# tenstack/batch-scheduler

Hardware: AMD Instinct MI355X
Metric: pod x node fit evals/sec (higher is better)
Workload: dtype int64; 1 GPU; cfg3/tail: 10000 pods / 2000 groups / 5000 nodes, 5 int64 lanes (cpu, mem, eph, pods, gpu), seed 20260921; stages=prefilter+filter+tally+ready, parallelism=single GPU

## Files before the change

### batch-scheduler_amd/capi.py

```python
from __future__ import annotations

import ctypes as C
import os

import numpy as np

from . import fitspec, soa

HERE = os.path.dirname(os.path.abspath(__file__))
LIB_PATH = os.path.join(os.environ.get("BS_LIB_DIR") or HERE, "libbsched.so")

KERNEL_COUNT = 8
KERNEL_PREPASS, KERNEL_LEADER, KERNEL_QUERY, KERNEL_TABLES, KERNEL_SCAN, KERNEL_RESOLVE, KERNEL_FILTER, KERNEL_TALLY = range(8)

ABI_SYMBOLS = [
    "bs_abi_version", "bs_strerror", "bs_last_error", "bs_create", "bs_destroy",
    "bs_nodes_load", "bs_fit_load", "bs_fit_build", "bs_fit_read", "bs_groups_load", "bs_groups_read", "bs_groups_apply", "bs_pods_map", "bs_pods_load",
    "bs_pods_apply", "bs_pods_count", "bs_pods_read", "bs_pods_apply_stats", "bs_filter_deny_stats", "bs_speculation_stats",
    "bs_nodes_apply", "bs_nodes_count", "bs_nodes_assume",
    "bs_cluster_fits", "bs_node_left", "bs_scan_prefix", "bs_cluster_total", "bs_filter_one", "bs_find_max_pg",
    "bs_batch_run", "bs_batch_sync", "bs_batch_read", "bs_batch_map", "bs_filter_rows_count", "bs_queue_order_load", "bs_queue_sort",
    "bs_shard_set", "bs_reduce_external", "bs_group_admit_devptr", "bs_group_admit_bind", "bs_stream", "bs_comm_unique_id", "bs_comm_init", "bs_batch_finish",
    "bs_timing_reset", "bs_timing_get", "bs_kernel_name", "bs_batch_stats_get",
    "bs_seq_run", "bs_nodes_read", "bs_first_reach_hint",
    "bs_nodes_load_flat", "bs_groups_load_flat", "bs_groups_read_flat", "bs_pods_load_flat", "bs_pods_apply_flat", "bs_pods_read_flat",
    "bs_batch_read_flat", "bs_seq_run_flat", "bs_fit_build_flat",
    "bs_bound_load", "bs_bound_count", "bs_preempt_run", "bs_bound_load_flat", "bs_preempt_run_flat",
    "bs_preempt_commit", "bs_bound_read", "bs_preempt_commit_flat",
    "bs_bound_pdb_set", "bs_preempt_pdb_read",
    "bs_bound_apply", "bs_bound_apply_flat", "bs_bound_ids", "bs_bound_dump",
    "bs_bound_nodes_apply",
    "bs_bound_apply_ex", "bs_bound_apply_ex_flat",
    "bs_pdb_load", "bs_pdb_members_append", "bs_pdb_allowed_apply", "bs_pdb_read",
    "bs_preempt_commit_gang", "bs_preempt_commit_gang_flat", "bs_preempt_gang_read",
    "bs_seq_expire", "bs_seq_expire_flat", "bs_seq_waiting_read",
    "bs_wait_load", "bs_wait_count", "bs_wait_ids", "bs_wait_read", "bs_wait_park", "bs_wait_release", "bs_wait_expire", "bs_wait_forget",
    "bs_wait_nodes_apply",
    "bs_groups_list_apply", "bs_groups_list_apply_flat",
    "bs_bound_bind",
    "bs_nominated_load", "bs_nominated_count", "bs_nominated_ids", "bs_nominated_read", "bs_nominated_apply", "bs_preempt_nominated_read",
    "bs_nominated_nodes_apply",
    "bs_preempt_cleared_read",
    "bs_seq_run_nominated", "bs_seq_run_nominated_flat", "bs_seq_nominated_read",
    "bs_seq_run_scored", "bs_seq_run_scored_flat", "bs_seq_score_read",
    "bs_seq_run_scored_nominated", "bs_seq_run_scored_nominated_flat",
]

SEQ_EXPIRE_DENY, SEQ_EXPIRE_ALL = 1, 2
WAIT_MAX = 1 << 24
NOM_MAX = 1 << 16
NOM_NONE = 0xFFFFFFFF
SCORE_WEIGHT_MAX = 65536

BS_BOUND_NODES = soa.BS_BOUND_NODES

PROTECTED_PHASES = (2, 5)


def group_protected(phases) -> np.ndarray:
    ph = np.asarray(phases, dtype=np.int64).reshape(-1)
    return np.isin(ph, PROTECTED_PHASES).astype(np.uint8)


def gang_order(pod_group, priority) -> np.ndarray:
    grp = np.asarray(pod_group, np.int64).reshape(-1)
    pri = np.asarray(priority, np.int64).reshape(-1)
    assert grp.shape == pri.shape
    first: dict = {}
    rank = np.zeros(grp.shape[0], np.int64)
    for i in range(grp.shape[0]):
        key = (int(pri[i]), int(grp[i])) if grp[i] >= 0 else (int(pri[i]), -1 - i)
        rank[i] = first.setdefault(key, i)
    return np.lexsort((np.arange(grp.shape[0]), rank, -pri)).astype(np.int64)


def gang_need(groups, waiting=None) -> np.ndarray:
    mm = np.asarray(groups.min_member, np.int64).reshape(-1)
    w = np.zeros_like(mm) if waiting is None else np.asarray(waiting, np.int64).reshape(-1)
    assert w.shape == mm.shape
    return np.clip(mm - np.asarray(groups.status_scheduled, np.int64).reshape(-1) - w, 0, None).astype(np.uint32)


class BsError(RuntimeError):
    def __init__(self, status: int, where: str, detail: str = ""):
        self.status = status
        super().__init__(f"{where}: status {status}" + (f" ({detail})" if detail else ""))


class Config(C.Structure):
    _fields_ = [("abi_version", C.c_uint32), ("device", C.c_int32), ("scalar_lanes", C.c_uint32),
                ("eph_gate", C.c_uint32), ("enable_timing", C.c_uint32), ("reserved", C.c_uint32 * 3)]


class NodeDelta(C.Structure):
    _fields_ = [("kind", C.c_uint32), ("index", C.c_uint32),
                ("allocatable", C.c_int64 * soa.MAX_LANES), ("requested", C.c_int64 * soa.MAX_LANES),
                ("allocatable_present", C.c_uint32), ("requested_present", C.c_uint32), ("flags", C.c_uint32),
                ("fit_default", C.c_uint32), ("n_fit_exceptions", C.c_uint32), ("fit_exceptions", C.c_uint32 * 8)]


class NodeRequest(C.Structure):
    _fields_ = [("index", C.c_uint32), ("requested_present", C.c_uint32), ("requested", C.c_int64 * soa.MAX_LANES)]


DELTA_UPDATE, DELTA_APPEND, DELTA_REMOVE = 0, 1, 2

# ... 24 lines not shown


class SeqExpireOut(C.Structure):
    _fields_ = [("n_groups", C.c_uint32), ("n_pods", C.c_uint32), ("group_cap", C.c_uint32), ("group", C.POINTER(C.c_uint32)),
                ("group_pods", C.POINTER(C.c_uint32)), ("group_earlier", C.POINTER(C.c_uint32)), ("pod_cap", C.c_uint32),
                ("pod", C.POINTER(C.c_uint32)), ("node", C.POINTER(C.c_uint32))]


_lib = None


class GroupsListDelta(C.Structure):
    _fields_ = [("n_remove", C.c_uint32), ("remove", C.POINTER(C.c_uint32)), ("n_update", C.c_uint32), ("update", C.POINTER(C.c_uint32)),
                ("rows", soa.GroupsStruct), ("n_append", C.c_uint32)]


class GroupsListOut(C.Structure):
    _fields_ = [("g_new", C.c_uint32), ("n_pods_missing", C.c_uint32), ("n_bound_missing", C.c_uint32), ("n_wait_dropped", C.c_uint32),
                ("wait_cap", C.c_uint32), ("wait_id", C.POINTER(C.c_uint32)), ("wait_node", C.POINTER(C.c_uint32)), ("wait_group", C.POINTER(C.c_int32))]


def load_library(path: str | None = None):
    global _lib
    if _lib is not None and path is None:
        return _lib
    p = path or LIB_PATH
    if not os.path.exists(p):
        raise BsError(-2, "load_library", f"{p} not built: run `python __graft_entry__.py build` (hipcc, gfx950)")
    L = C.CDLL(p)
    vp, u32, i32, u8 = C.c_void_p, C.c_uint32, C.c_int32, C.c_uint8
    P = C.POINTER
    L.bs_abi_version.restype = u32
    L.bs_strerror.restype = C.c_char_p
    L.bs_strerror.argtypes = [C.c_int]
    L.bs_last_error.restype = C.c_char_p
    L.bs_last_error.argtypes = [vp]
    L.bs_kernel_name.restype = C.c_char_p
    L.bs_kernel_name.argtypes = [u32]
    L.bs_create.argtypes = [P(Config), P(vp)]
    L.bs_destroy.argtypes = [vp]
    L.bs_nodes_load.argtypes = [vp, P(soa.NodesStruct)]
    L.bs_fit_load.argtypes = [vp, u32, P(u32)]
    L.bs_fit_build.argtypes = [vp, P(fitspec.NodeLabelsStruct), P(fitspec.FitTemplatesStruct)]
    L.bs_fit_read.argtypes = [vp, P(u32)]
    L.bs_groups_load.argtypes = [vp, P(soa.GroupsStruct)]
    L.bs_groups_read.argtypes = [vp, P(soa.GroupsStruct)]
    L.bs_groups_apply.argtypes = [vp, P(soa.GroupDelta), u32]
    L.bs_filter_rows_count.argtypes = [vp, P(u32)]
    L.bs_pods_load.argtypes = [vp, P(soa.PodsStruct)]
    L.bs_pods_map.argtypes = [vp, u32, P(soa.PodsStruct)]
    L.bs_pods_apply.argtypes = [vp, P(soa.PodsDeltaStruct)]
    L.bs_pods_count.argtypes = [vp, P(u32)]
    L.bs_pods_apply_stats.argtypes = [vp, P(C.c_uint64), P(C.c_uint64)]
    L.bs_filter_deny_stats.argtypes = [vp, P(C.c_uint64)]
    L.bs_speculation_stats.argtypes = [vp, P(C.c_uint64), P(C.c_uint64)]
    L.bs_pods_read.argtypes = [vp, P(soa.PodsOutStruct)]
    L.bs_queue_order_load.argtypes = [vp, u32, P(u32)]
    L.bs_queue_sort.argtypes = [vp, u32, P(i32), P(i32), P(C.c_int64), P(u32)]
    L.bs_nodes_apply.argtypes = [vp, P(NodeDelta), u32]
    L.bs_nodes_count.argtypes = [vp, P(u32)]
    L.bs_nodes_assume.argtypes = [vp, P(NodeRequest), u32]
    L.bs_cluster_fits.argtypes = [vp, u32, C.c_float, P(C.c_int64), u32, P(u8), P(u32)]
    L.bs_node_left.argtypes = [vp, u32, C.c_float, P(C.c_int64), P(u32)]
    L.bs_scan_prefix.argtypes = [vp, u32, C.c_float, P(C.c_int64), P(u32), P(u32), P(u32)]
    L.bs_cluster_total.argtypes = [vp, u32, P(C.c_int64), P(u32)]
    L.bs_filter_one.argtypes = [vp, i32, P(C.c_int64), u32, i32, u32, P(u8), P(u8)]
    L.bs_find_max_pg.argtypes = [vp, P(i32), P(u32), P(u8)]
    L.bs_batch_run.argtypes = [vp, u32]
    L.bs_batch_sync.argtypes = [vp]
    L.bs_batch_read.argtypes = [vp, P(soa.BatchOutStruct)]
    L.bs_batch_map.argtypes = [vp, P(soa.BatchViewStruct)]
    L.bs_shard_set.argtypes = [vp, u32, u32]
    L.bs_group_admit_devptr.argtypes = [vp, P(vp), P(u32)]
    L.bs_reduce_external.argtypes = [vp, u32]
    L.bs_first_reach_hint.argtypes = [vp, u32]
    L.bs_group_admit_bind.argtypes = [vp, vp]
    L.bs_stream.argtypes = [vp, P(vp)]
    L.bs_comm_unique_id.argtypes = [P(u8)]
    L.bs_comm_init.argtypes = [vp, P(u8), u32, u32]
    L.bs_batch_finish.argtypes = [vp]
    L.bs_timing_reset.argtypes = [vp]
    L.bs_timing_get.argtypes = [vp, P(Timing)]
    L.bs_batch_stats_get.argtypes = [vp, P(BatchStats)]
    L.bs_seq_run.argtypes = [vp, u32, P(SeqOut)]
    L.bs_nodes_read.argtypes = [vp, P(C.c_int64), P(u32)]
    L.bs_bound_load.argtypes = [vp, P(soa.BoundStruct)]
    L.bs_bound_count.argtypes = [vp, P(u32)]
    L.bs_preempt_run.argtypes = [vp, u32, u32, P(u32), P(i32), P(u8), u32, P(soa.PreemptOutStruct)]
    L.bs_bound_load_flat.argtypes = [vp, u32, P(u32), P(i32), P(C.c_int64), P(i32), P(C.c_int64), P(u32)]
    L.bs_preempt_run_flat.argtypes = [vp, u32, u32, P(u32), P(i32), P(u8), u32, P(i32), P(u32), P(u32), P(u32), P(i32), P(C.c_int64), P(C.c_int64)]
    L.bs_preempt_commit.argtypes = [vp, u32, u32, P(u32), P(i32), P(u8), u32, u32, P(soa.PreemptOutStruct)]
    L.bs_bound_read.argtypes = [vp, P(u32), P(u32)]
    L.bs_bound_pdb_set.argtypes = [vp, u32, P(u8)]
    L.bs_bound_apply.argtypes = [vp, P(soa.BoundDeltaStruct), P(u32)]
    L.bs_bound_apply_flat.argtypes = [vp, u32, P(u32), u32, P(u32), P(i32), P(C.c_int64), P(i32), P(C.c_int64), P(u32), P(u8), P(u32)]
    L.bs_bound_apply_ex.argtypes = [vp, P(soa.BoundDeltaStruct), u32, P(u32)]
    L.bs_bound_apply_ex_flat.argtypes = [vp, u32, u32, P(u32), u32, P(u32), P(i32), P(C.c_int64), P(i32), P(C.c_int64), P(u32), P(u8), P(u32)]
    L.bs_bound_ids.argtypes = [vp, P(u32)]
    L.bs_bound_nodes_apply.argtypes = [vp, u32, P(u32), P(u32), u32, P(u32), P(u32)]
    L.bs_bound_dump.argtypes = [vp, P(i32), P(C.c_int64), P(i32), P(C.c_int64), P(u32), P(u8)]
    L.bs_preempt_pdb_read.argtypes = [vp, u32, P(u32)]
    L.bs_pdb_load.argtypes = [vp, u32, P(i32), u32, P(u32), P(u32)]
    L.bs_pdb_members_append.argtypes = [vp, u32, u32, P(u32), P(u32)]
    L.bs_pdb_allowed_apply.argtypes = [vp, u32, P(u32), P(i32)]
    L.bs_pdb_read.argtypes = [vp, P(u32), P(u32), P(i32), P(u32)]
    L.bs_preempt_commit_flat.argtypes = [vp, u32, u32, P(u32), P(i32), P(u8), u32, u32, P(i32), P(u32), P(u32), P(u32), P(i32), P(C.c_int64),
                                         P(C.c_int64)]
    L.bs_preempt_commit_gang.argtypes = [vp, u32, u32, P(u32), P(i32), P(u8), P(u32), u32, u32, P(soa.PreemptOutStruct)]
    L.bs_preempt_commit_gang_flat.argtypes = [vp, u32, u32, P(u32), P(i32), P(u8), P(u32), u32, u32, P(i32), P(u32), P(u32), P(u32), P(i32),
                                              P(C.c_int64), P(C.c_int64)]
    L.bs_preempt_gang_read.argtypes = [vp, u32, P(u8), u32, P(u32)]
    L.bs_seq_expire.argtypes = [vp, u32, P(u32), u32, P(SeqExpireOut)]
    L.bs_seq_expire_flat.argtypes = [vp, u32, P(u32), u32, u32, P(u32), P(u32), P(u32), u32, P(u32), P(u32), P(u32)]
    L.bs_seq_waiting_read.argtypes = [vp, u32, P(i32)]
    L.bs_wait_load.argtypes = [vp, u32, P(u32), P(i32), P(C.c_int64), P(u32)]
    L.bs_wait_count.argtypes = [vp, P(u32)]
    L.bs_wait_ids.argtypes = [vp, P(u32)]
    L.bs_wait_read.argtypes = [vp, P(u32), P(u32), P(i32), P(C.c_int64), P(u32)]
    L.bs_wait_park.argtypes = [vp, u32, P(u32), P(u32), P(u32), P(u32)]
    L.bs_wait_release.argtypes = [vp, u32, P(u32), u32, P(u32), P(u32), P(u32), P(u32)]
    L.bs_wait_expire.argtypes = [vp, u32, P(u32), u32, u32, P(u32), P(u32), P(u32), P(u32), P(u32)]
    L.bs_wait_forget.argtypes = [vp, u32, P(u32), P(u32)]
    L.bs_wait_nodes_apply.argtypes = [vp, u32, P(u32), P(u32), u32, P(u32), P(u32), P(i32), P(u32)]
    L.bs_groups_list_apply.argtypes = [vp, P(GroupsListDelta), P(GroupsListOut)]
    L.bs_groups_list_apply_flat.argtypes = [vp, u32, P(u32), u32, P(u32), u32, P(u32), P(u32), P(u32), P(u8), P(u32), P(C.c_int64), P(u32), P(C.c_uint64),
                                            u32, u32, P(u32), P(u32), P(i32), P(u32)]
    L.bs_nominated_load.argtypes = [vp, u32, P(u32), P(i32), P(C.c_int64), P(u32)]
    L.bs_nominated_count.argtypes = [vp, P(u32)]
    L.bs_nominated_ids.argtypes = [vp, P(u32)]
    L.bs_nominated_read.argtypes = [vp, P(u32), P(u32), P(i32), P(C.c_int64), P(u32)]
    L.bs_nominated_apply.argtypes = [vp, u32, P(u32), u32, P(u32), P(u32), P(i32), P(u32)]
    L.bs_preempt_nominated_read.argtypes = [vp, u32, P(u32)]
    L.bs_preempt_cleared_read.argtypes = [vp, u32, P(u32), P(u32), P(i32), P(u32), P(u32)]
    L.bs_nominated_nodes_apply.argtypes = [vp, u32, P(u32), P(u32), u32, P(u32), P(u32), P(i32), P(u32)]
    L.bs_bound_bind.argtypes = [vp, u32, P(u32), u32, P(u32), P(i32), P(C.c_int64), P(u8), P(u32), P(u32)]
    L.bs_seq_run_nominated.argtypes = [vp, u32, u32, P(i32), P(u32), P(SeqOut)]
    L.bs_seq_run_nominated_flat.argtypes = [vp, u32, u32, P(i32), P(u32), P(u8), P(u32), P(i32), P(i32), u32, P(u32), P(u32), P(C.c_int64), P(C.c_int64),
                                            P(C.c_int64), P(u8)]
    L.bs_seq_nominated_read.argtypes = [vp, u32, P(u32), P(u32), P(u32), P(u32)]
    L.bs_seq_run_scored.argtypes = [vp, u32, P(SeqScore), P(SeqOut)]
    L.bs_seq_run_scored_flat.argtypes = [vp, u32, u32, u32, u32, P(u8), P(u32), P(i32), P(i32), u32, P(u32), P(u32), P(C.c_int64), P(C.c_int64),
                                         P(C.c_int64), P(u8)]
    L.bs_seq_score_read.argtypes = [vp, u32, P(u32), P(u32)]
    L.bs_seq_run_scored_nominated.argtypes = [vp, u32, u32, P(i32), P(u32), P(SeqScore), P(SeqOut)]
    L.bs_seq_run_scored_nominated_flat.argtypes = [vp, u32, u32, P(i32), P(u32), u32, u32, u32, P(u8), P(u32), P(i32), P(i32), u32, P(u32), P(u32), P(C.c_int64),
                                                   P(C.c_int64), P(C.c_int64), P(u8)]
    for name in ABI_SYMBOLS:
        fn = getattr(L, name)
        if fn.restype is C.c_int:
            fn.restype = C.c_int
    if path is None:
        _lib = L
    return L


def _i64p(a):
    return a.ctypes.data_as(C.POINTER(C.c_int64))


def _u32p(a):
    return a.ctypes.data_as(C.POINTER(C.c_uint32))


class Context:

    def __init__(self, scalar_lanes: int = 0, eph_gate: int = 1, device: int = 0, enable_timing: int = 0):
# ... 725 lines not shown
    def bound_nodes_apply(self, kind, index, dropped_cap: int = 0):
        kv = np.ascontiguousarray(np.asarray(kind, np.uint32).reshape(-1))
        iv = np.ascontiguousarray(np.asarray(index, np.uint32).reshape(-1))
        assert kv.size == iv.size
        ids = np.zeros(max(int(dropped_cap), 1), np.uint32)
        nd = C.c_uint32()
        self._chk(self._lib.bs_bound_nodes_apply(self._h, int(kv.size), _u32p(kv) if kv.size else None, _u32p(iv) if iv.size else None,
                                                 int(dropped_cap), _u32p(ids) if dropped_cap else None, C.byref(nd)), "bs_bound_nodes_apply")
        return int(nd.value), ids[: min(int(nd.value), int(dropped_cap))].copy()

    def pdb_load(self, allowed, member_off, member, b: int | None = None):
        al = np.ascontiguousarray(allowed, np.int32).reshape(-1)
        off = np.ascontiguousarray(member_off, np.uint32).reshape(-1)
        mem = np.ascontiguousarray(member, np.uint32).reshape(-1)
        b = max(off.size - 1, 0) if b is None else int(b)
        self._chk(self._lib.bs_pdb_load(self._h, int(al.size), al.ctypes.data_as(C.POINTER(C.c_int32)) if al.size else None, b,
                                        _u32p(off) if off.size else None, _u32p(mem) if mem.size else None), "bs_pdb_load")

    def pdb_members_append(self, first_id: int, member_off, member):
        off = np.ascontiguousarray(member_off, np.uint32).reshape(-1)
        mem = np.ascontiguousarray(member, np.uint32).reshape(-1)
        self._chk(self._lib.bs_pdb_members_append(self._h, int(first_id), max(off.size - 1, 0), _u32p(off) if off.size else None,
                                                  _u32p(mem) if mem.size else None), "bs_pdb_members_append")

    def pdb_allowed_apply(self, index, value):
        ix = np.ascontiguousarray(index, np.uint32).reshape(-1)
        va = np.ascontiguousarray(value, np.int32).reshape(-1)
        assert ix.size == va.size
        self._chk(self._lib.bs_pdb_allowed_apply(self._h, int(ix.size), _u32p(ix) if ix.size else None,
                                                 va.ctypes.data_as(C.POINTER(C.c_int32)) if va.size else None), "bs_pdb_allowed_apply")

    def pdb_read(self) -> dict:
        n, cov = C.c_uint32(0), C.c_uint32(0)
        self._chk(self._lib.bs_pdb_read(self._h, C.byref(n), C.byref(cov), None, None), "bs_pdb_read")
        nodes = C.c_uint32(0)
        self._chk(self._lib.bs_nodes_count(self._h, C.byref(nodes)), "bs_nodes_count")
        al, nv = np.zeros(max(n.value, 1), np.int32), np.zeros(max(nodes.value, 1), np.uint32)
        self._chk(self._lib.bs_pdb_read(self._h, None, None, al.ctypes.data_as(C.POINTER(C.c_int32)), _u32p(nv)), "bs_pdb_read")
        return dict(n_pdb=int(n.value), covered=int(cov.value), allowed=al[: n.value], node_violating=nv[: nodes.value])

    def bound_dump(self) -> dict:
        b = self.bound_count()
        n = max(b, 1)
        prio, start, grp = np.zeros(n, np.int32), np.zeros(n, np.int64), np.zeros(n, np.int32)
        req, pres, pdb = np.zeros((self.L, n), np.int64), np.zeros(n, np.uint32), np.zeros(n, np.uint8)
        self._chk(self._lib.bs_bound_dump(self._h, prio.ctypes.data_as(C.POINTER(C.c_int32)), _i64p(start), grp.ctypes.data_as(C.POINTER(C.c_int32)),
                                          _i64p(req), _u32p(pres), pdb.ctypes.data_as(C.POINTER(C.c_uint8))), "bs_bound_dump")
        return dict(priority=prio[:b], start_ns=start[:b], group=grp[:b], req=req[:, :b], req_present=pres[:b], pdb=pdb[:b])

    def set_shard(self, rank: int, nranks: int):
        self._chk(self._lib.bs_shard_set(self._h, rank, nranks), "bs_shard_set")

    def reduce_external(self, on: bool = True):
        self._chk(self._lib.bs_reduce_external(self._h, 1 if on else 0), "bs_reduce_external")

    def first_reach_hint(self, local_index: int):
        self._chk(self._lib.bs_first_reach_hint(self._h, int(local_index) & 0xFFFFFFFF), "bs_first_reach_hint")

    def admit_devptr(self):
        p, n = C.c_void_p(), C.c_uint32(0)
        self._chk(self._lib.bs_group_admit_devptr(self._h, C.byref(p), C.byref(n)), "bs_group_admit_devptr")
        return int(p.value or 0), int(n.value)

    def bind_admit(self, dptr: int | None):
        self._chk(self._lib.bs_group_admit_bind(self._h, C.c_void_p(dptr or 0)), "bs_group_admit_bind")

    def stream(self) -> int:
        p = C.c_void_p()
        self._chk(self._lib.bs_stream(self._h, C.byref(p)), "bs_stream")
        return int(p.value or 0)

    def comm_init(self, uid: bytes, rank: int, nranks: int):
        buf = (C.c_uint8 * 128).from_buffer_copy(uid)
        self._chk(self._lib.bs_comm_init(self._h, buf, rank, nranks), "bs_comm_init")

    def timing_reset(self):
        self._chk(self._lib.bs_timing_reset(self._h), "bs_timing_reset")

    def timing(self) -> dict:
        t = Timing()
        self._chk(self._lib.bs_timing_get(self._h, C.byref(t)), "bs_timing_get")
        return {self._lib.bs_kernel_name(i).decode(): (float(t.total_ms[i]), int(t.launches[i])) for i in range(KERNEL_COUNT)}

    def stats_arm(self):
        s = BatchStats()
        self._chk(self._lib.bs_batch_stats_get(self._h, C.byref(s)), "bs_batch_stats_get")

    def stats(self, stages: int = soa.STAGE_ALL) -> dict:
        self.stats_arm()
        self.run(stages)
        self.sync()
        return self.stats_read()

    def stats_read(self) -> dict:
        s = BatchStats()
        self._chk(self._lib.bs_batch_stats_get(self._h, C.byref(s)), "bs_batch_stats_get")
        return {k: int(getattr(s, k)) for k, _ in BatchStats._fields_}


def comm_unique_id() -> bytes:
    lib = load_library()
    buf = (C.c_uint8 * 128)()
    rc = lib.bs_comm_unique_id(buf)
    if rc != 0:
        raise BsError(rc, "bs_comm_unique_id")
    return bytes(buf)
```

### batch-scheduler_amd/csrc/bs_ctx.hpp

```cpp
#pragma once
#include <rccl/rccl.h>

#include <algorithm>
#include <cstring>
#include <functional>
#include <string>
#include <vector>

#include "bs_carve.hpp"
#include "bs_hostmem.hpp"
#include "bs_kernels.hpp"
#include "bs_lanes.hpp"
#include "bs_layouts.hpp"
#include "bs_pod_ranges.hpp"
#include "bs_preempt_clear_list.hpp"

namespace bs {

struct EventPair { hipEvent_t a, b; uint32_t id; };

inline size_t align256(size_t x) { return (x + 255) & ~(size_t)255; }
template <class T>
T* at(T* p, size_t n) { return p ? p + n : nullptr; }

// ... 128 lines not shown
  uint64_t n_applies = 0, n_rederives = 0;
  OutLayout olay;

  DevBuf d_first_elig, d_first_owner, d_first_reject, d_first_pod, d_cap_epoch;
  DevBuf d_epoch, d_nepochs, d_leader_epoch, d_panic_epoch;
  DevBuf d_tcode, d_stage, d_leader_raw, d_first_row, d_first_row64, d_scan_rec, d_feas_rec, d_chunk_rec, d_qreq_s, d_qflags_s, d_qpos;
  DevBuf d_needed, d_qcount, d_ticket, d_desc;
  bool scratch_armed = false;
  bool side_ready = false;
  DevBuf d_tables, d_kp, d_stats, d_fparams, d_fflags, d_chunk_tot, d_blk_scratch, d_gmax, d_chunk_kp;
  DevBuf d_cls_slots, d_cls_rep, d_cls_id, d_qtab_s, d_fu_slot, d_uparams, d_uflags, d_uclaim, d_fu_bitmap, d_fu_feas;
  DevBuf d_nodew;
  bool batch_void = false;
  uint32_t tp_tmin = 768;
  bool no_nodew = false;
  uint32_t slot_keep = 0xFFFFFFFFu;
  uint32_t cls_cap = 0, hash_keep = 0x7FFFFFFFu, n_nominres = 0, scan_slots_cap = 0, filter_slots_cap = 0;
  DevBuf d_fl_bitmap, d_admit, d_ready, d_gcount, d_admit64, d_own_start;
  bool owner_ready = false;
  DevBuf d_order_rank, d_sort;
  uint32_t order_g = 0;
  DevBuf d_gstat, d_pair_next, d_pair_firstq, d_first_reach, d_qstamp_s, d_fast_reject, d_epoch_group;
  bool pairs_ready = false;
  bool bitmap_valid = false;
  bool last_fast = false;
  bool batch_since_pods = false;
  size_t off_hfeas = 0, off_htag = 0;
  uint32_t hstride = 0;
  int32_t host_tag = 0;
  bool last_host_out = false;
  uint32_t no_fast = 0;
  DevBuf d_run_of_epoch, d_run_leader, d_gslot, d_gfirstq;
  bool epochs_ready = false, einfo_pending = false;
  int32_t einfo_tag = 0;
  uint32_t h_R = 0, h_eflags = 0, no_epoch = 0;
  uint32_t last_chain = 0;
  uint32_t last_rows = 0;
  DevBuf d_sq;
  DevBuf d_seq;
  bool seq_wait_valid = false;
  Piece<unsigned long long> seq_o_wait;
  Piece<uint32_t> seq_o_head, seq_o_nwait;
  Piece<int32_t> seq_o_node;
  bool seq_nom_valid = false;
  std::vector<uint32_t> seq_nom_id, seq_nom_pod, seq_nom_node;
  DevBuf d_seq_score;
  bool seq_score_valid = false;
  uint32_t seq_score_p = 0;
  DevBuf d_sexp;
  DevBuf d_sexp_nodes;
  uint32_t sexp_n = 0, sexp_l = 0;
  bool sexp_clean = false;
  bool have_wait = false;
  uint32_t wait_w = 0, wait_ids = 0;
  uint32_t wait_n = 0, wait_g = 0;
  DevBuf d_wait[2];
  uint32_t wait_cap[2] = {0, 0};
  uint32_t wait_cur = 0;
  DevBuf d_wait_scr;
  DevBuf d_wait_nodes;
  DevBuf d_wait_gmark, d_wait_imark;
  bool wait_nodes_clean = false, wait_gmark_clean = false, wait_imark_clean = false;
  uint32_t table_slots = 0, table_mcap = 0;

  uint32_t rank = 0, nranks = 1;
  bool reduce_external = false;
  uint32_t* ext_admit = nullptr;
  int32_t sop_leader0 = -1;
  uint32_t last_stages = 0;
  uint64_t batch_seq = 0;
  uint32_t stamp_ctr = 1, key_seq = 1;
  bool rekey_pending = false;
  bool batch_pending_finish = false;
  bool groups_launch_pending = false;
  DeltaPack pending_dp{};
  uint32_t no_fuse_final = 0;
  uint32_t tp_filter = 6;
  uint32_t tp_share = 0;
  uint32_t tp_fwaves = 0;
  bool filter_waves_env = false;
  uint32_t tp_split = 0;
  int fused_blocks_resident = -1;
  int step_a_resident[2] = {-1, -1};
  uint32_t step_a_form = 3;
  bool step_a_on = true;
  uint32_t step_shares = 8;
  uint32_t test_timeout_after = 0;
  uint32_t test_pc_chunk_nodes = 0;
  uint32_t tk_pods = 0, tk_tab = 0;
  uint32_t tk_p1 = 0, tk_done = 0;
  bool pod_ranges_on = true;
  bool ranges_valid = false;
  uint32_t nranges = 0;
  PodRanges h_ranges;
  std::vector<uint32_t> h_pod_ranges;
  DevBuf d_pod_ranges;
  bool last_step_a = false;
  uint32_t scan_share_override = 0, no_fuse_filter = 0, early_forced = 0, target_waves = 8192, filter_waves = 8192, collect_stats = 0;
  uint32_t general_waves = 4096;
  bs_batch_stats stats{};

  std::vector<EventPair> events;
  size_t events_used = 0;
  bs_timing timing{};

  void* rccl_handle = nullptr;
  void* comm = nullptr;
  decltype(&ncclAllReduce) rccl_allreduce = nullptr;
  decltype(&ncclCommDestroy) rccl_destroy = nullptr;
  uint32_t launches = 0;
  DevBuf d_fd_event, d_fd_in, d_fd_flag;
  bool fd_on = false;
  bool fd_active = false;
  uint32_t first_reach_hint = 0xFFFFFFFFu;
  bool fd_unsynced = false;
  bool fd_in_live = false;
  uint32_t fd_iter = 0, fd_stages = 0, fd_seq_inv = 0;
  uint64_t n_fd_reruns = 0;
  bool have_bound = false;
  uint32_t bound_b = 0, bound_n = 0;
  int32_t bound_max_group = -1;
  DevBuf d_bound, d_pre;
  DevBuf d_bound2;
  BoundLayout blay{};
  uint32_t bound_ids = 0;
  std::vector<uint32_t> pre_npv;
  bool have_pre_npv = false;
  std::vector<uint8_t> gang_voided;
  std::vector<uint32_t> gang_placed;
  bool have_gang = false;
  bool have_pdb = false;
  uint32_t pdb_n = 0, pdb_covered = 0, pdb_members = 0;
  DevBuf d_pdb_allowed, d_pdb_moff, d_pdb_member;
  bool have_nom = false;
  uint32_t nom_w = 0, nom_ids = 0;
  uint32_t nom_n = 0;
  DevBuf d_nom[2];
  uint32_t nom_cap[2] = {0, 0};
  uint32_t nom_ncap[2] = {0, 0};
  uint32_t nom_cur = 0;
  std::vector<uint32_t> nom_live;
  std::vector<uint32_t> pre_nom;
  bool have_pre_nom = false;
  ClearedRows pre_clr;

  Stream stream;
  Stream stream3;
  Event ev_query, ev_filter;
  PinnedBuf<int32_t> h_info{PinWait::None, hipHostMallocMapped | hipHostMallocCoherent};
  PinnedBuf<> h_gstage{PinWait::Event};
  PinnedBuf<> h_glstage{PinWait::Stream};
  PinnedBuf<> h_stage{PinWait::Event};
  PinnedBuf<> h_dstage{PinWait::Stream};
  PinnedBuf<> h_nstage{PinWait::Event};
  PinnedBuf<> h_pdbstage{PinWait::Stream};
  PinnedBuf<> h_rstage;
  PinnedBuf<> h_hout{PinWait::None, hipHostMallocMapped | hipHostMallocCoherent};
  PinnedBuf<uint64_t> h_hrows{PinWait::None, hipHostMallocMapped | hipHostMallocCoherent};
};

inline int32_t hinfo_get(const bs_ctx* c, HInfo w) { return static_cast<volatile const int32_t*>(c->h_info.p)[w]; }
inline void hinfo_set(bs_ctx* c, HInfo w, int32_t v) { static_cast<volatile int32_t*>(c->h_info.p)[w] = v; }
inline int32_t* hinfo_at(const bs_ctx* c, HInfo w) { return c->h_info.p ? c->h_info.p + w : nullptr; }

#define HIPCHK(ctx, call)                                                                         \
  do {                                                                                            \
    hipError_t _e = (call);                                                                       \
    if (_e != hipSuccess) {                                                                       \
      (ctx)->last_error = std::string(#call) + ": " + hipGetErrorString(_e);                      \
      return BS_ERR_HIP;                                                                          \
    }                                                                                             \
  } while (0)
#define LAUNCHCHK(ctx, id)                                                                         \
  do {                                                                                             \
    hipError_t _e = hipGetLastError();                                                             \
    if (_e != hipSuccess) {                                                                        \
      (ctx)->last_error = std::string("launch of kernel group '") + kKernelNames[id] + "': " + hipGetErrorString(_e); \
      return BS_ERR_HIP;                                                                           \
    }                                                                                              \
  } while (0)
// ... 1 lines not shown
```

### batch-scheduler_amd/csrc/bs_fast.hpp

```cpp
#pragma once

#include "bs_kernels.hpp"
#include "bs_filter_t.hpp"

#ifdef BS_NT_TABLES
#define BS_TBL_STORE(p, v) __builtin_nontemporal_store((v), (p))
#else
#define BS_TBL_STORE(p, v) (*(p) = (v))
#endif
namespace bs {

template <bool INL = false>
__device__ __forceinline__ void arm_tally(const GroupsDev& gr, const BatchDev& b, const BatchParams& prm, uint32_t i, uint32_t nthreads);

__device__ __forceinline__ const uint8_t* range_glocal(const BatchDev& b) { return reinterpret_cast<const uint8_t*>(b.pod_ranges); }
__device__ __forceinline__ const uint32_t* range_start(const BatchDev& b, uint32_t G) { return b.pod_ranges + (G + 3u) / 4u; }
__device__ __forceinline__ const uint32_t* range_lfirst(const BatchDev& b, uint32_t G, uint32_t pod_blocks) { return range_start(b, G) + pod_blocks + 1u; }
__device__ __forceinline__ bool range_local_on(const BatchDev& b, const BatchParams& prm) {
  return b.pod_ranges && prm.do_tally && prm.do_ready && !prm.filter_deny;
}

#if BS_EMIT_MAIN
__global__ void k_pods_prep(unsigned long long* tables, uint32_t ntab, uint32_t* gstat, uint32_t ngstat, uint32_t* kcount, uint32_t* gcount, uint32_t G) {
  const uint32_t t = blockIdx.x * blockDim.x + threadIdx.x, nt = gridDim.x * blockDim.x;
// ... 466 lines not shown
    LeaderPre lp{};
    const bool have = gr.g != 0 && leaders[s] >= 0;
    if (have) leader_pre_load(gr, leaders[s], sh, lp);
    Res ms;
    res_zero(ms, sh);
    if (have && lp.have_mr) res_add(ms, lp.mr, sh, gate);
    uint32_t ff = (have && lp.have_mr) ? 1u : 0u;
#pragma unroll
    for (uint32_t q = 0; q < BS_MAX_SCALARS; ++q)
      if (q < sh.S() && (ms.present & (1u << q)) && ms.v[4 + q] != 0) ff |= 2u;
    const unsigned long long holds = __ballot(l[0] >= ms.v[0] && l[1] >= ms.v[1] && l[2] >= ms.v[2] && l[3] >= ms.v[3]);
    if (stores) {
      b.nodew[nodew_pair(stride, s, w)] = ok;
      b.nodew[nodew_pair(stride, s, w) + 1] = ~holds;
    }
    if (blk == 0 && threadIdx.x == 0) {
#pragma unroll
      for (int j = 0; j < 4; ++j) b.nodew[nodew_ref_lane(stride, s, j)] = (uint64_t)ms.v[j];
      b.nodew[nodew_ref_flags(stride, s)] = ff;
    }
  }
}

template <int TS>
__global__ __launch_bounds__(kTblChunk) void k_fast_query_tables(PodsDev pods, GroupsDev gr, NodesDev nd, BatchDev b, BatchDev bt, BatchParams prm,
                                                                 const TableDesc* forced, uint32_t nchunks, uint32_t query_blocks) {
  BS_STAMP(1, 0);
  if (blockIdx.x < query_blocks) fast_query_thread<TS>(pods, gr, b, prm, blockIdx.x * kTblChunk + threadIdx.x, query_blocks * kTblChunk);
  else if (blockIdx.x < query_blocks + nchunks) tables_local_fast<TS>(nd, bt, prm, forced, blockIdx.x - query_blocks);
  else node_words_block<TS>(gr, nd, b, prm, blockIdx.x - query_blocks - nchunks);
  BS_STAMP(1, 7);
}

template <int NL>
__device__ __forceinline__ unsigned long long rows_cover(unsigned long long m, const int64_t (&a)[BS_MAX_LANES], const int64_t (&r)[BS_MAX_LANES]) {
  asm volatile("s_mov_b64 exec, %[m]\n\tv_cmpx_ge_i64 vcc, %[a0], %[r0]\n\tv_cmpx_ge_i64 vcc, %[a1], %[r1]\n\tv_cmpx_ge_i64 vcc, %[a2], %[r2]\n\t"
               "v_cmpx_ge_i64 vcc, %[a3], %[r3]\n\ts_mov_b64 %[m], exec\n\ts_mov_b64 exec, -1"
               : [m] "+s"(m)
               : [a0] "v"(a[0]), [r0] "v"(r[0]), [a1] "v"(a[1]), [r1] "v"(r[1]), [a2] "v"(a[2]), [r2] "v"(r[2]), [a3] "v"(a[3]), [r3] "v"(r[3])
               : "vcc");
#pragma unroll
  for (int j = 4; j < NL; ++j)
    asm volatile("s_mov_b64 exec, %[m]\n\tv_cmpx_ge_i64 vcc, %[a], %[r]\n\ts_mov_b64 %[m], exec\n\ts_mov_b64 exec, -1" : [m] "+s"(m) : [a] "v"(a[j]), [r] "v"(r[j]) : "vcc");
  return m;
}
#ifndef BS_SCAN_BALLOT
#define BS_SCAN_BALLOT 1
#endif
constexpr uint32_t kSpinBound = 1u << 18;
__device__ __forceinline__ void test_chaos_delay() {
#ifdef BS_TEST_CHAOS
  uint32_t h = (blockIdx.x + 1u) * 2654435761u ^ (uint32_t)wall_clock64() * 40503u;
  h ^= h >> 15; h *= 2246822519u; h ^= h >> 13;
  for (uint32_t s = 0; s < (h & 15u); ++s) __builtin_amdgcn_s_sleep(127);
#endif
}
__device__ __forceinline__ bool step_wait(const uint32_t* word, uint32_t base, uint32_t need, int32_t* h_err) {
  uint32_t spins = 0;
  while ((uint32_t)(ld_agent(word) - base) < need) {
    __builtin_amdgcn_s_sleep(1);
    if (++spins > kSpinBound) { if (h_err) __hip_atomic_store(h_err, 1, __ATOMIC_RELAXED, __HIP_MEMORY_SCOPE_SYSTEM); return false; }
  }
  return true;
}
constexpr uint32_t kScanRecChunks = 64;
constexpr uint32_t kFeasRecGroups = 32;
constexpr uint32_t kRecStride = 32;
constexpr uint32_t kTkSlots = 32, kTkTab = 48, kTkP1 = 64, kTkDone = 64 + 16 * 16, kTkWays = 16, kTkWords = 64 + 2 * 16 * 16;
__device__ __forceinline__ void spread_add(uint32_t* words, uint32_t who) {
  (void)__hip_atomic_fetch_add(&words[16u * (who % kTkWays)], 1u, __ATOMIC_RELAXED, __HIP_MEMORY_SCOPE_AGENT);
}
__device__ __forceinline__ bool spread_wait(const uint32_t* words, uint32_t base, uint32_t need, int32_t* h_err) {
  uint32_t spins = 0;
  for (;;) {
    uint32_t v = lane_id() < (int)kTkWays ? ld_agent(&words[16u * (uint32_t)lane_id()]) : 0u;
#pragma unroll
    for (int o = 1; o < (int)kTkWays; o <<= 1) v += (uint32_t)__shfl_xor((int)v, o);
    v = (uint32_t)__builtin_amdgcn_readfirstlane((int)v);
    if ((uint32_t)(v - base) >= need) return true;
    __builtin_amdgcn_s_sleep(4);
    if (++spins > kSpinBound) { if (h_err && lane_id() == 0) __hip_atomic_store(h_err, 1, __ATOMIC_RELAXED, __HIP_MEMORY_SCOPE_SYSTEM); return false; }
  }
}
template <int TS, bool REGS = false>
__device__ __forceinline__ void table_scan_block(const NodesDev& nd, const BatchDev& b, const BatchParams& prm, const TableDesc* forced, uint32_t chunk, uint32_t nchunks,
                                                 uint32_t share, uint32_t nshares, uint32_t pod_blocks, uint32_t tk_pods0, uint32_t tk_tab0, const GroupsDev& gr,
                                                 const int64_t* ckeys, const uint32_t* cpres, uint32_t kcap, bool direct = false, uint32_t forced_cls = 0) {
  __shared__ unsigned long long s_wtot[BS_MAX_LANES][4];
  __shared__ uint32_t s_kp[BS_MAX_SCALARS];
  __shared__ unsigned long long s_off[BS_MAX_LANES];
  __shared__ uint32_t s_kpg[BS_MAX_SCALARS];
  __shared__ int64_t s_req[kStepSlotsMax][BS_MAX_LANES];
  __shared__ uint32_t s_qf[kStepSlotsMax];
  __shared__ uint32_t s_first[kStepSlotsMax];
  BS_STAMP(2, 0);
  const Shape<TS> sh(prm.S);
  const uint32_t L = sh.L(), S = sh.S(), LP = prm.LP;
  const uint32_t k = chunk * kTblChunk + threadIdx.x;
  const bool in_range = REGS ? k < nd.n : k < nd.m;
  const uint32_t n = REGS ? (in_range ? k : 0u) : (in_range ? nd.kmap[k] : 0u);
  const TableDesc d = REGS ? TableDesc{forced_cls, 0.7f} : *forced;
  const uint32_t fw = nd.fit[(size_t)d.cls * nd.fit_words + (n >> 5)];
  const uint8_t fl = nd.flags[n];
  const bool valid = in_range && (!REGS || !(fl & BS_NODE_SKIP_MASK));
  const uint32_t ap = nd.apres[n], rp = nd.rpres[n];
  int64_t al[BS_MAX_LANES], rq[BS_MAX_LANES];
#pragma unroll
  for (uint32_t j = 0; j < BS_MAX_LANES; ++j) {
    if (j < L) {
      al[j] = nd.alloc[(size_t)j * nd.stride + n];
      rq[j] = nd.req[(size_t)j * nd.stride + n];
    }
  }
  const uint32_t K = prm.k_host ? prm.k_host : *b.kclass;
  const uint32_t per = (K + nshares - 1u) / nshares, s_lo = share * per, s_hi = min(K, s_lo + per);
  Res raw;
  int32_t leader0 = -1;
  uint8_t panic0 = 0;
  LeaderPre lp0{};
  if constexpr (REGS) {
    const uint32_t cc = s_lo + threadIdx.x < s_hi ? s_lo + threadIdx.x : 0u;
#pragma unroll
    for (uint32_t j = 0; j < BS_MAX_LANES; ++j)
      if (j < L) raw.v[j] = ckeys[(size_t)j * kcap + cc];
    raw.present = cpres[cc];
    leader0 = b.leader_epoch[0];
    panic0 = b.panic_epoch[0];
    if (gr.g) leader_pre_load(gr, leader0, sh, lp0);
  }
  const bool fit = valid && ((fw >> (n & 31u)) & 1u) && !(fl & BS_NODE_TAINT_ERR);
  const uint32_t pres = fit ? (ap & rp) : 0u;
  if (threadIdx.x < BS_MAX_SCALARS) s_kp[threadIdx.x] = BS_INF;
  for (uint32_t t = threadIdx.x; t < kStepSlotsMax; t += kTblChunk) s_first[t] = BS_INF;
  unsigned long long incl[BS_MAX_LANES];
  const int w = wave_id();
#pragma unroll
  for (uint32_t j = 0; j < BS_MAX_LANES; ++j) {
    incl[j] = 0;
    if (j < L) {
      const bool live = fit && (j < 4 || (pres & (1u << (j - 4)))) && !(j == BS_LANE_EPH && !prm.eph_gate);
      const unsigned long long left = live ? (unsigned long long)wsub(scale_f32(al[j], d.pct), rq[j]) : 0ull;
      incl[j] = wave_incl_scan_add_u64(left);
      if (lane_id() == 63) s_wtot[j][w] = incl[j];
    }
  }
  __syncthreads();
#pragma unroll
  for (uint32_t s2 = 0; s2 < BS_MAX_SCALARS; ++s2) {
    if (s2 < S) {
      const unsigned long long mk = __ballot(valid && (pres & (1u << s2)));
      if (mk && lane_id() == 0) atomicMin(&s_kp[s2], chunk * kTblChunk + (uint32_t)(threadIdx.x & ~63u) + (uint32_t)(__ffsll((long long)mk) - 1));
    }
  }
#pragma unroll
  for (uint32_t j = 0; j < BS_MAX_LANES; ++j) {
    if (j < L) {
      unsigned long long off = 0, tot = 0;
#pragma unroll
      for (int i = 0; i < 4; ++i) {
        const unsigned long long x = s_wtot[j][i];
        if (i < w) off += x;
        tot += x;
      }
      incl[j] += off;
      if (threadIdx.x == 0 && share == 0) {
        if constexpr (REGS) {
          const unsigned long long tag = (unsigned long long)prm.seq_inv << 32;
          st_pub<true>(&b.chunk_rec[(size_t)chunk * kRecStride + 2u * j], tag | (uint32_t)tot);
          st_pub<true>(&b.chunk_rec[(size_t)chunk * kRecStride + 2u * j + 1u], tag | (uint32_t)(tot >> 32));
        } else {
          st_pub<true>(&b.chunk_tot[(size_t)chunk * 16 + j], tot);
        }
      }
    }
  }
  __syncthreads();
  __shared__ uint32_t s_ok;
  if constexpr (REGS) {
    if (share == 0 && threadIdx.x < S) st_pub<true>(&b.chunk_rec[(size_t)chunk * kRecStride + 16u + threadIdx.x], ((unsigned long long)prm.seq_inv << 32) | s_kp[threadIdx.x]);
    BS_STAMP(2, 1);
  } else {
    if (share == 0 && threadIdx.x < 16) st_pub<true>(&b.chunk_kp[(size_t)chunk * 16 + threadIdx.x], threadIdx.x < BS_MAX_SCALARS ? s_kp[threadIdx.x] : BS_INF);
    asm volatile("s_waitcnt vmcnt(0)" ::: "memory");
    __syncthreads();
    BS_STAMP(2, 1);
    if (threadIdx.x == 0 && share == 0) (void)__hip_atomic_fetch_add(&b.ticket[kTkTab], 1u, __ATOMIC_RELAXED, __HIP_MEMORY_SCOPE_AGENT);
  }
  if constexpr (REGS) {
    const uint32_t t = s_lo + threadIdx.x;
    if (t < s_hi) {
      uint32_t qf = 0x80000000u;
      Res q;
      res_zero(q, sh);
      if (leader0 >= 0 && !panic0) {
        Res cur;
        res_zero(cur, sh);
        res_add(cur, raw, sh, prm.eph_gate);
        qf = class_scan_query(cur, lp0, sh, prm.eph_gate, q);
      }
      s_qf[threadIdx.x] = qf;
#pragma unroll
      for (uint32_t j = 0; j < BS_MAX_LANES; ++j)
        if (j < L) s_req[threadIdx.x][j] = q.v[j];
    }
  }
  if constexpr (!REGS) {
    if (threadIdx.x == 0) s_ok = (step_wait(&b.ticket[kTkTab], tk_tab0, nchunks, b.h_err) && step_wait(&b.ticket[kTkSlots], tk_pods0, pod_blocks, b.h_err)) ? 1u : 0u;
    __syncthreads();
    BS_STAMP(2, 2);
    if (!s_ok) return;
  }
  {
    const uint32_t ch = (uint32_t)lane_id();
    unsigned long long cv[BS_MAX_LANES];
    uint32_t ckp[BS_MAX_SCALARS];
    if constexpr (REGS) {
      if (w == 0) {
        const uint32_t tagw = prm.seq_inv;
        const unsigned long long* rec = b.chunk_rec + (size_t)(ch < nchunks ? ch : 0u) * kRecStride;
        bool ok = false;
        for (uint32_t spins = 0;; ++spins) {
          unsigned long long lo[BS_MAX_LANES], hi[BS_MAX_LANES], kw[BS_MAX_SCALARS];
#pragma unroll
          for (uint32_t j = 0; j < BS_MAX_LANES; ++j)
            if (j < L) { lo[j] = ld_agent64(&rec[2u * j]); hi[j] = ld_agent64(&rec[2u * j + 1u]); }
// ... 47 lines not shown
    if (w == 0) {
#pragma unroll
      for (uint32_t j = 0; j < BS_MAX_LANES; ++j) {
        if (j < L) {
          const unsigned long long incl_c = wave_incl_scan_add_u64(cv[j]);
          const unsigned long long mine = bcast64(incl_c - cv[j], (int)(chunk & 63u));
          if (ch == 0) s_off[j] = mine;
        }
      }
#pragma unroll
      for (uint32_t s2 = 0; s2 < BS_MAX_SCALARS; ++s2) {
        if (s2 < S) {
          const uint32_t mn = wave_min_u32(ckp[s2]);
          if (ch == 0) s_kpg[s2] = mn;
        }
      }
    }
    if (!REGS && t < s_hi) {
      if (stp != prm.stamp || tab != 0) qf = 0x80000000u;
      s_qf[threadIdx.x] = qf;
#pragma unroll
      for (uint32_t j = 0; j < BS_MAX_LANES; ++j)
        if (j < L) s_req[threadIdx.x][j] = (int64_t)rv[j];
    }
  }
  __syncthreads();
  if constexpr (REGS) {
    if (!s_ok) return;
  }
  int64_t fin[BS_MAX_LANES];
  uint32_t keyrow = 0;
#pragma unroll
  for (uint32_t j = 0; j < BS_MAX_LANES; ++j) {
    fin[j] = 0;
    if (j < L) fin[j] = (int64_t)(incl[j] + s_off[j]);
  }
#pragma unroll
  for (uint32_t s2 = 0; s2 < BS_MAX_SCALARS; ++s2)
    if (s2 < S && k >= s_kpg[s2]) keyrow |= 1u << s2;
  BS_STAMP(2, 3);
  const uint32_t nmine = s_hi > s_lo ? s_hi - s_lo : 0u;
  const uint32_t smask = S ? ((1u << S) - 1u) : 0u;
  const uint32_t row0 = chunk * kTblChunk + ((uint32_t)w << 6);
  for (uint32_t t0 = 0; t0 < nmine; t0 += 4u) {
    uint32_t qf[4];
    int64_t r[4][BS_MAX_LANES];
#pragma unroll
    for (uint32_t u = 0; u < 4; ++u) {
      const uint32_t t = min(t0 + u, nmine - 1u);
      qf[u] = t0 + u < nmine ? s_qf[t] : 0x80000000u;
#pragma unroll
      for (uint32_t j = 0; j < BS_MAX_LANES; ++j) r[u][j] = j < L ? s_req[t][j] : 0;
    }
#pragma unroll
    for (uint32_t u = 0; u < 4; ++u) {
      const uint32_t nab = ~(qf[u] >> 16) & smask;
      unsigned long long m = (qf[u] & 0x80000000u) ? 0ull : __ballot(valid && (nab & ~keyrow) == 0u);
      static_assert(TS >= 0 && TS <= 4, "k_fast_step_a is instantiated for 0..4 scalar lanes (bs_step_geom.hpp: step_a_possible)");
#if BS_SCAN_BALLOT
#pragma unroll
      for (uint32_t j = 0; j < 4u + (uint32_t)TS; ++j) m &= __ballot(fin[j] >= r[u][j]);
#else
      m = rows_cover<4 + TS>(m, fin, r[u]);
#endif
      if (m && lane_id() == 0) atomicMin(&s_first[t0 + u], row0 + (uint32_t)(__ffsll((long long)m) - 1));
    }
  }
  __syncthreads();
  BS_STAMP(2, 4);
  if constexpr (REGS) {
    if (direct) {
      for (uint32_t t = threadIdx.x; t < nmine; t += kTblChunk)
        st_pub<true>(&b.scan_rec[(size_t)chunk * kStepSlotsMax + s_lo + t], ((unsigned long long)prm.seq_inv << 32) | s_first[t]);
    } else {
      for (uint32_t t = threadIdx.x; t < nmine; t += kTblChunk)
        if (s_first[t] != BS_INF) atomicMin(&b.first_row64[s_lo + t], ((unsigned long long)prm.seq_inv << 32) | s_first[t]);
    }
    BS_STAMP(2, 7);
    return;
  }
  for (uint32_t t = threadIdx.x; t < nmine; t += kTblChunk) {
    if (s_first[t] == BS_INF) continue;
    atomicMin(&b.first_row[s_lo + t], s_first[t]);
  }
  BS_STAMP(2, 7);
}

__device__ __forceinline__ void step_filter_split(uint32_t K, uint32_t W, uint32_t target_waves, uint32_t& tiles, uint32_t& bpw, uint32_t& nchunk) {
  tiles = (2u * K + 63u) / 64u;
  uint32_t nsplit = max(1u, target_waves / max(tiles, 1u));
  nsplit = min(nsplit, max((W + 1u) / 2u, 1u));
  bpw = max(2u, (((W + nsplit - 1u) / nsplit + 1u) / 2u) * 2u);
  nchunk = (W + bpw - 1u) / bpw;
  if ((nchunk + 3u) / 4u > kFeasRecGroups) {
    bpw = ((W + 4u * kFeasRecGroups - 1u) / (4u * kFeasRecGroups) + 1u) / 2u * 2u;
    nchunk = (W + bpw - 1u) / bpw;
  }
}
template <int TS>
__device__ __forceinline__ void step_filter_block(const GroupsDev& gr, const NodesDev& nd, const BatchDev& b, const BatchParams& prm, const int64_t* ckeys,
                                                  const uint32_t* cpres, uint32_t kcap, uint32_t target_waves, uint32_t ustride, uint32_t bx, uint32_t nblocks,
                                                  bool direct, uint32_t tk_slots0, uint32_t slot_producers) {
  __shared__ uint32_t s_cnt[4][64];
  BS_STAMP_AT(4, 0, bx);
  const Shape<TS> sh(prm.S);
  const uint32_t gate = prm.eph_gate, K = prm.k_host ? prm.k_host : (uint32_t)__builtin_amdgcn_readfirstlane((int)*b.kclass), U = 2u * K;
  const uint32_t W = (nd.n + 63u) / 64u;
  if (!U || !W) return;
  uint32_t tiles, bpw, nchunk;
  step_filter_split(K, W, target_waves, tiles, bpw, nchunk);
  const uint32_t groups = (nchunk + 3u) / 4u;
  const int32_t leader0 = b.leader_epoch[0];
  LeaderPre lp0{}, lp1{};
  const bool two = prm.sop_leader0 >= 0 && prm.sop_leader0 != leader0;
  if (gr.g) {
    leader_pre_load(gr, leader0, sh, lp0);
    if (two) leader_pre_load(gr, prm.sop_leader0, sh, lp1); else lp1 = lp0;
  }
  bool waited = false;
  for (uint32_t bi = bx; bi < tiles * groups; bi += nblocks) {
    const uint32_t tile = bi % tiles, group = bi / tiles, chunk = group * 4u + (uint32_t)wave_id();
    const uint32_t src = tile * 64u + (uint32_t)lane_id();
    const bool second = src >= K;
    const uint32_t c = src < U ? (second ? src - K : src) : 0u;
    uint32_t cnt = 0;
    if (chunk < nchunk) {
      Res raw;
#pragma unroll
      for (uint32_t j = 0; j < BS_MAX_LANES; ++j)
        if (j < sh.L()) raw.v[j] = ckeys[(size_t)j * kcap + c];
      raw.present = cpres[c];
      Res cur;
      res_zero(cur, sh);
      res_add(cur, raw, sh, gate);
      LeaderPre lp = lp0;
      if (second) lp = lp1;
      const bool on = src < U && (second ? prm.sop_leader0 >= 0 : leader0 >= 0) && lp.have_mr;
      int64_t R[4], M[4];
      const uint32_t ff = filter_slot_values(cur, lp, sh, gate, R, M);
      filter_item<2, 4, true, true>(nd, b, U, ustride, tile, chunk * bpw, min(W, chunk * bpw + bpw), 0u,
                                    on ? (ff | ((uint32_t)BS_FL_EVALUATED << 8)) : ((uint32_t)BS_FL_NOT_RUN << 8), R, M, &cnt);
    }
    s_cnt[wave_id()][lane_id()] = cnt;
    BS_STAMP_AT(4, 1, bx);
    if (direct && b.h_rows) asm volatile("s_waitcnt vmcnt(0)" ::: "memory");
    __syncthreads();
    BS_STAMP_AT(4, 2, bx);
    if (wave_id() == 0 && src < U) {
      const uint32_t sum = s_cnt[0][lane_id()] + s_cnt[1][lane_id()] + s_cnt[2][lane_id()] + s_cnt[3][lane_id()];
      if (direct) {
        st_pub<true>(&b.feas_rec[(size_t)group * (2u * kStepSlotsMax) + src], ((unsigned long long)prm.seq_inv << 32) | sum);
      } else {
        if (!waited) { (void)step_wait(&b.ticket[kTkSlots], tk_slots0, slot_producers, b.h_err); waited = true; }
        if (sum) atomicAdd(&b.fu_feas[src], sum);
      }
    }
    __syncthreads();
  }
  BS_STAMP_AT(4, 7, bx);
}

template <int TS>
__device__ __forceinline__ void class_slots_block(const GroupsDev& gr, const BatchDev& b, const BatchParams& prm, const int64_t* ckeys, const uint32_t* cpres,
                                                  uint32_t kcap, uint32_t blk, bool zero_feas) {
  const Shape<TS> sh(prm.S);
#ifdef BS_TEST_OLD_ZERO
// ... 361 lines not shown
    else
      tally_tail<true>(gr, b, prm, grouped, grouped ? (uint32_t)gi0 : 0u, admit, nblocks);
  }
  BS_STAMP(3, 7);
}

template <int S>
__global__ __launch_bounds__(256) void k_fast_scan_filter(PodsDev pods, NodesDev nd, BatchDev bt, BatchParams prm, uint32_t m, uint32_t jcap,
                                                          uint32_t scan_blocks, uint32_t filter_waves, uint32_t ustride) {
  __shared__ int64_t s_rows[4][64][4 + S];
  if (blockIdx.x < scan_blocks)
    scan_loop<S, true, 1>(bt, prm, m, jcap, 0u, 0u, 1u, blockIdx.x, scan_blocks, s_rows[wave_id()]);
  else
    filter_loop<2>(pods, nd, bt, filter_waves, 1u, ustride, prm.collect_stats, blockIdx.x - scan_blocks, gridDim.x - scan_blocks, prm.stamp, 2u * prm.k_host);
}
template <int S>
__global__ __launch_bounds__(256) void k_fast_scan(BatchDev bt, BatchParams prm, uint32_t m, uint32_t jcap) {
  __shared__ int64_t s_rows[4][64][4 + S];
  scan_loop<S, true, 1>(bt, prm, m, jcap, 0u, 0u, 1u, blockIdx.x, gridDim.x, s_rows[wave_id()]);
}
template <int PU, bool DB>
__global__ __launch_bounds__(256) void k_fast_filter(PodsDev pods, NodesDev nd, BatchDev bt, BatchParams prm, uint32_t filter_waves, uint32_t ustride) {
  filter_loop<2, PU, DB>(pods, nd, bt, filter_waves, 1u, ustride, prm.collect_stats, blockIdx.x, gridDim.x, prm.stamp, 2u * prm.k_host);
}
#if BS_EMIT_FAST
__global__ __launch_bounds__(256) __attribute__((amdgpu_waves_per_eu(7))) void k_fast_filter_w7(PodsDev pods, NodesDev nd, BatchDev bt, BatchParams prm, uint32_t filter_waves,
                                                                                                uint32_t ustride) {
  filter_loop<2, 2, false>(pods, nd, bt, filter_waves, 1u, ustride, prm.collect_stats, blockIdx.x, gridDim.x, prm.stamp, 2u * prm.k_host);
}
#endif
#if BS_EMIT_FAST
__global__ __launch_bounds__(256) void k_fast_filter_t(NodesDev nd, BatchDev bt, BatchParams prm, uint32_t filter_waves, uint32_t ustride, uint32_t by_tile) {
  filter_loop_t<false>(nd, bt, filter_waves, ustride, prm.collect_stats, blockIdx.x, gridDim.x, prm.stamp, 2u * prm.k_host, by_tile);
}
#endif
template <int S>
__global__ __launch_bounds__(256) __attribute__((amdgpu_waves_per_eu(S <= 1 ? 4 : 1))) void k_fast_scan_filter_t(NodesDev nd, BatchDev bt, BatchParams prm, uint32_t m, uint32_t jcap, uint32_t scan_blocks,
                                                            uint32_t filter_waves, uint32_t ustride, uint32_t form) {
  __shared__ int64_t s_rows[4][64][4 + S];
  const uint32_t filter_first = form & 1u, by_tile = form & 2u;
  const uint32_t filter_blocks = gridDim.x - scan_blocks;
  const bool is_scan = filter_first ? blockIdx.x >= filter_blocks : blockIdx.x < scan_blocks;
  BS_STAMP(2, 0);
  if (is_scan)
    scan_loop<S, true, 1>(bt, prm, m, jcap, 0u, 0u, 1u, filter_first ? blockIdx.x - filter_blocks : blockIdx.x, scan_blocks, s_rows[wave_id()]);
  else
    filter_loop_t<true>(nd, bt, filter_waves, ustride, prm.collect_stats, filter_first ? blockIdx.x : blockIdx.x - scan_blocks, filter_blocks, prm.stamp, 2u * prm.k_host, by_tile);
  BS_STAMP(2, 7);
}
#if BS_EMIT_MAIN
__global__ __launch_bounds__(256) void k_fast_final(PodsDev pods, GroupsDev gr, NodesDev nd, BatchDev b, BatchParams prm, uint32_t query_blocks) {
  fast_final_block(pods, gr, nd, b, prm, query_blocks, blockIdx.x, gridDim.x, 0u);
}
#endif

template <int S>
__global__ __launch_bounds__(256) void k_fast_scan_filter_final(PodsDev pods, GroupsDev gr, NodesDev nd, BatchDev b, BatchDev bt, BatchParams prm, uint32_t m,
                                                                uint32_t jcap, uint32_t scan_blocks, uint32_t filter_blocks, uint32_t filter_waves,
                                                                uint32_t ustride, uint32_t query_blocks) {
  __shared__ int64_t s_rows[4][64][4 + S];
  const uint32_t producers = scan_blocks + filter_blocks;
  test_chaos_delay();
#ifdef BS_TEST_LATE_ROLE_B
  {
    const int role = blockIdx.x < scan_blocks ? 0 : blockIdx.x < producers ? 1 : 2;
    if (role == BS_TEST_LATE_ROLE_B) for (int spin = 0; spin < 20; ++spin) __builtin_amdgcn_s_sleep(127);
  }
#endif
  if (blockIdx.x < producers) {
    BS_STAMP(2, 0);
    if (blockIdx.x < scan_blocks)
      scan_loop<S, true, 2>(bt, prm, m, jcap, 0u, 0u, 1u, blockIdx.x, scan_blocks, s_rows[wave_id()]);
    else
      filter_loop<2>(pods, nd, bt, filter_waves, 1u, ustride, prm.collect_stats, blockIdx.x - scan_blocks, filter_blocks, prm.stamp, 2u * prm.k_host);
    asm volatile("s_waitcnt vmcnt(0)" ::: "memory");
    __syncthreads();
    if (threadIdx.x == 0) (void)__hip_atomic_fetch_add(&b.ticket[1], 1u, __ATOMIC_RELAXED, __HIP_MEMORY_SCOPE_AGENT);
    BS_STAMP(2, 7);
    return;
  }
  fast_final_block(pods, gr, nd, b, prm, query_blocks, blockIdx.x - producers, gridDim.x - producers, producers);
}

template <int TS, bool WHOLE>
__global__ __launch_bounds__(kTblChunk) void k_fast_step_a(PodsDev pods, GroupsDev gr, NodesDev nd, BatchDev b, BatchDev bt, BatchParams prm, const TableDesc* forced,
                                                           uint32_t nchunks, uint32_t query_blocks, uint32_t nshares, uint32_t filter_blocks, uint32_t filter_waves,
                                                           uint32_t ustride, uint32_t tk_pods0, uint32_t tk_tab0, uint32_t param_blocks, const int64_t* ckeys,
                                                           const uint32_t* cpres, uint32_t kcap, uint32_t tk_p1, uint32_t tk_done, uint32_t forced_cls) {
  BS_STAMP(1, 0);
  test_chaos_delay();
  const uint32_t tb = nchunks * nshares;
#ifdef BS_TEST_LATE_ROLE
  {
    const int role = blockIdx.x < query_blocks ? 0 : blockIdx.x < query_blocks + param_blocks ? 1 : blockIdx.x < query_blocks + param_blocks + tb ? 2 : 3;
    if (role == BS_TEST_LATE_ROLE) for (int spin = 0; spin < 20; ++spin) __builtin_amdgcn_s_sleep(127);
  }
#endif
  const uint32_t producers = param_blocks ? param_blocks : query_blocks;
  const bool direct = query_blocks <= kGatherDirectBlocks;
  if (blockIdx.x < query_blocks) {
    if constexpr (WHOLE) {
      const uint32_t p0 = b.pod_ranges ? range_start(b, gr.g)[blockIdx.x] : blockIdx.x * kTblChunk;
      const uint32_t p1 = b.pod_ranges ? range_start(b, gr.g)[blockIdx.x + 1u] : pods.p;
      fast_query_thread<TS, false, false, true>(pods, gr, b, prm, p0 + threadIdx.x, query_blocks * kTblChunk, p1, blockIdx.x * kTblChunk + threadIdx.x);
      asm volatile("s_waitcnt vmcnt(0)" ::: "memory");
      __syncthreads();
      if (threadIdx.x == 0) spread_add(&b.ticket[kTkP1], blockIdx.x);
      fast_final_block<true>(pods, gr, nd, b, prm, query_blocks, blockIdx.x, query_blocks, nchunks, tk_p1, filter_waves, tk_done, tb + filter_blocks, p0, p1);
    } else if (param_blocks) {
      fast_query_thread<TS, false, false>(pods, gr, b, prm, blockIdx.x * kTblChunk + threadIdx.x, query_blocks * kTblChunk);
    } else {
      fast_query_thread<TS, true>(pods, gr, b, prm, blockIdx.x * kTblChunk + threadIdx.x, query_blocks * kTblChunk);
      BS_STAMP(1, 4);
      asm volatile("s_waitcnt vmcnt(0)" ::: "memory");
      __syncthreads();
      BS_STAMP(1, 5);
      if (threadIdx.x == 0) (void)__hip_atomic_fetch_add(&b.ticket[kTkSlots], 1u, __ATOMIC_RELAXED, __HIP_MEMORY_SCOPE_AGENT);
    }
  } else if (blockIdx.x < query_blocks + param_blocks) {
    class_slots_block<TS>(gr, b, prm, ckeys, cpres, kcap, blockIdx.x - query_blocks, !(WHOLE && direct));
  } else if (blockIdx.x < query_blocks + param_blocks + tb) {
    const uint32_t x = blockIdx.x - query_blocks - param_blocks;
    table_scan_block<TS, WHOLE>(nd, bt, prm, forced, x / nshares, nchunks, x % nshares, nshares, producers, tk_pods0, tk_tab0, gr, ckeys, cpres, kcap, direct, forced_cls);
    if constexpr (WHOLE) {
      if (!direct) {
        asm volatile("s_waitcnt vmcnt(0)" ::: "memory");
        __syncthreads();
        if (threadIdx.x == 0) spread_add(&b.ticket[kTkDone], blockIdx.x);
      }
    }
  } else if constexpr (WHOLE) {
    step_filter_block<TS>(gr, nd, bt, prm, ckeys, cpres, kcap, filter_waves, ustride, blockIdx.x - query_blocks - param_blocks - tb, filter_blocks, direct, tk_pods0, producers);
    if (!direct) {
      asm volatile("s_waitcnt vmcnt(0)" ::: "memory");
      __syncthreads();
      if (threadIdx.x == 0) spread_add(&b.ticket[kTkDone], blockIdx.x);
    }
  } else {
    __shared__ uint32_t s_go;
    if (threadIdx.x == 0) {
      s_go = step_wait(&b.ticket[kTkSlots], tk_pods0, producers, b.h_err) ? 1u : 0u;
      __builtin_amdgcn_fence(__ATOMIC_ACQUIRE, "agent");
    }
    __syncthreads();
    if (!s_go) return;
    filter_loop<2>(pods, nd, bt, filter_waves, 1u, ustride, prm.collect_stats, blockIdx.x - query_blocks - param_blocks - tb, filter_blocks, prm.stamp, 2u * prm.k_host);
  }
  BS_STAMP(1, 7);
}


template <int TS>
__global__ __launch_bounds__(kTblChunk) void k_tables_local_nofix(NodesDev nd, BatchDev b, BatchParams prm, uint32_t nchunks, uint32_t cstride,
                                                                  uint32_t gstride) {
  const uint32_t slot = blockIdx.x;
  if (!b.needed[slot]) return;
  BatchDev bt = b;
  bt.tables = b.tables + (size_t)slot * prm.mcap * prm.LP;
  bt.kp = b.kp + (size_t)slot * 16;
  bt.chunk_tot = b.chunk_tot + (size_t)slot * cstride * 16;
  bt.chunk_kp = b.chunk_kp + (size_t)slot * cstride * 16;
  bt.gmax = b.gmax + (size_t)slot * gstride * prm.LP;
  const TableDesc d = table_desc(slot, prm.C, nullptr);
  tables_local_fast<TS>(nd, bt, prm, &d, blockIdx.y);
}

#if BS_EMIT_MAIN
__global__ __launch_bounds__(kLeaderBlock) void k_leader_scan(GroupsDev gr, BatchDev b) {
  __shared__ unsigned long long s_w[kLeaderBlock / 64];
  __shared__ uint32_t s_p[kLeaderBlock / 64];
  __shared__ unsigned long long s_carry;
  __shared__ uint32_t s_pcarry, s_nexact, s_exact[64];
  const uint32_t E1 = *b.nepochs;
  auto key_of = [&](uint32_t g, bool& panic) -> unsigned long long {
    if (gr.flags[g] & BS_GROUP_SCHEDULED_LATCH) return 0ull;
    const uint32_t f = leader_finished(gr, g, panic);
    return (((unsigned long long)f + 1ull) << 31) | (unsigned long long)(0x7FFFFFFFu - g);
  };
  unsigned long long k0 = 0;
  bool p0 = false;
  for (uint32_t g = threadIdx.x; g < gr.g; g += kLeaderBlock)
    if (b.cap_epoch[g] == 0u) { const unsigned long long k = key_of(g, p0); k0 = k > k0 ? k : k0; }
  {
    const unsigned long long m = block_max_u64(k0, s_w);
    const unsigned long long anyp = __ballot(p0);
    if (lane_id() == 0) s_p[wave_id()] = anyp ? 1u : 0u;
    __syncthreads();
    if (threadIdx.x == 0) {
      uint32_t pp = 0;
      for (int w = 0; w < kLeaderBlock / 64; ++w) pp |= s_p[w];
      s_carry = m;
      s_pcarry = pp;
      s_nexact = 0;
    }
    __syncthreads();
  }
  for (uint32_t base = 0; base < E1; base += kLeaderBlock) {
    const uint32_t e = base + threadIdx.x;
    unsigned long long k = 0;
    bool pn = false;
    if (e >= 1 && e < E1) k = key_of(b.epoch_group[e], pn);
    uint32_t pv = pn ? 1u : 0u;
#pragma unroll
    for (int o = 1; o < 64; o <<= 1) {
      const unsigned long long u = __shfl_up(k, o);
      const uint32_t q = (uint32_t)__shfl_up((int)pv, o);
      if (lane_id() >= o) { k = u > k ? u : k; pv |= q; }
    }
    __syncthreads();
    if (lane_id() == 63) { s_w[wave_id()] = k; s_p[wave_id()] = pv; }
    __syncthreads();
    unsigned long long off = s_carry;
    uint32_t poff = s_pcarry;
    for (int w = 0; w < wave_id(); ++w) { off = s_w[w] > off ? s_w[w] : off; poff |= s_p[w]; }
    k = off > k ? off : k;
// ... 46 lines not shown
```

### batch-scheduler_amd/csrc/bs_launch.hpp

```cpp
#pragma once
#include <hip/hip_runtime.h>
#include <stdint.h>

#include "bs_kernels.hpp"
#include "bs_lanes.hpp"

namespace bs {

struct FastLaunch {
  hipStream_t stream;
  uint32_t S, M, P, filter_waves, filter_slots_cap, tp_filter;
  int device;
  uint32_t filter_split = 0;
};
void launch_fast_bc(const FastLaunch& c, dim3 grid, const PodsDev& pd, const GroupsDev& gr, const NodesDev& nd, const BatchDev& b, const BatchDev& bt,
                    const BatchParams& prm, uint32_t nseg, uint32_t scan_blocks, uint32_t filter_blocks);
void launch_fast_b(const FastLaunch& c, dim3 grid, const PodsDev& pd, const NodesDev& nd, const BatchDev& bt, const BatchParams& prm, uint32_t nseg,
                   uint32_t scan_blocks);
void launch_fast_scan(const FastLaunch& c, dim3 grid, const BatchDev& bt, const BatchParams& prm, uint32_t nseg);
void launch_fast_bt(const FastLaunch& c, dim3 grid, const NodesDev& nd, const BatchDev& bt, const BatchParams& prm, uint32_t nseg, uint32_t scan_blocks);
void launch_fast_filter(const FastLaunch& c, dim3 grid, const PodsDev& pd, const NodesDev& nd, const BatchDev& bt, const BatchParams& prm);
int fused_residency_query(const FastLaunch& c);
void launch_fast_step_a(const FastLaunch& c, dim3 grid, const PodsDev& pd, const GroupsDev& gr, const NodesDev& nd, const BatchDev& b, const BatchDev& bt,
                        const BatchParams& prm, const TableDesc* forced, uint32_t nchunks, uint32_t query_blocks, uint32_t nshares, uint32_t filter_blocks,
                        uint32_t tk_pods0, uint32_t tk_tab0, uint32_t param_blocks, const int64_t* ckeys, const uint32_t* cpres, uint32_t kcap,
                        uint32_t whole, uint32_t tk_p1, uint32_t tk_done, uint32_t forced_cls);
int step_a_residency_query(const FastLaunch& c, bool whole);

}
```

### batch-scheduler_amd/csrc/bs_step_geom.hpp

```cpp
#pragma once
#include <cstdint>

#ifndef BS_GATHER_DIRECT
#define BS_GATHER_DIRECT 8
#endif

namespace bs {

constexpr int kTblChunk = 256;
constexpr uint32_t kStepSlotsMax = 256;
constexpr uint32_t kGatherDirectBlocks = BS_GATHER_DIRECT;

constexpr uint32_t cdiv(uint32_t a, uint32_t b) { return (a + b - 1) / b; }
constexpr uint32_t geom_min(uint32_t a, uint32_t b) { return a < b ? a : b; }
constexpr uint32_t geom_max(uint32_t a, uint32_t b) { return a > b ? a : b; }

constexpr uint32_t filter_blocks(uint32_t waves, uint32_t slot_tiles, uint32_t W) {
  return cdiv(geom_min(waves, slot_tiles * geom_max(1u, cdiv(W, 2u))), 4u);
}

struct StepIn {
  uint32_t P, G, N, M, S, W;
  uint32_t k_host, k_bound, h_K;
  bool kinfo_pending;
  uint32_t step_a_form, step_shares;
  bool step_a_on;
  uint32_t filter_waves;
  bool filter_waves_env;
  uint32_t tp_filter, tp_share, tp_fwaves, tp_tmin;
  uint32_t target_waves, scan_share;
  uint32_t nranks;
  bool run_filter, dirs_ready;
  bool ranges_valid;
  uint32_t nranges;
  bool whole_bufs;
  bool no_fuse_final, no_nodew, have_nodew;
  bool collect_stats;
  int enable_timing;
};

constexpr uint32_t table_chunks(uint32_t M) { return geom_max(1u, cdiv(M, 256u)); }

constexpr uint32_t step_k(const StepIn& in) {
  return !in.kinfo_pending ? in.k_host : ((in.step_a_form >= 3u && in.dirs_ready) ? in.k_bound : 0u);
}

constexpr bool step_a_possible(const StepIn& in, uint32_t k, uint32_t nchunks) {
  return in.step_a_on && !in.no_fuse_final && k > 0 && k <= kStepSlotsMax && nchunks <= 64 && in.M > 0 && in.P > 0 && !in.collect_stats &&
         in.enable_timing < 2 && in.S <= 4;
}

struct StepAPlan {
  bool ready;
  bool whole, ranges;
  uint32_t qb, pb, nchunks, nshares, fblocks, grid;
  uint32_t launches;
  uint32_t tk_pods, tk_tab, tk_p1, tk_done;
};

constexpr StepAPlan step_a_plan(const StepIn& in, uint32_t K) {
  StepAPlan p{};
  p.nshares = geom_max(1u, geom_min(in.step_shares, cdiv(K, 8u)));
  p.fblocks = in.run_filter ? filter_blocks(in.filter_waves, cdiv(2u * K, 64u), in.W) : 0u;
  p.pb = (in.step_a_form >= 2u && in.dirs_ready) ? cdiv(K, kTblChunk) : 0u;
  const uint32_t nch_nodes = geom_max(1u, cdiv(in.N, 256u));
  p.whole = in.step_a_form >= 3u && p.pb && nch_nodes <= 64u && in.whole_bufs;
  p.nchunks = p.whole ? nch_nodes : table_chunks(in.M);
  p.ranges = p.whole && in.ranges_valid && in.nranges;
  p.qb = p.ranges ? in.nranges : cdiv(in.P, kTblChunk);
  p.grid = p.qb + p.pb + p.nchunks * p.nshares + p.fblocks;
  p.ready = !in.kinfo_pending || p.whole;
  p.launches = p.whole ? 1u : 2u;
  p.tk_pods = p.pb ? p.pb : p.qb;
  p.tk_tab = p.whole ? 0u : p.nchunks;
  p.tk_p1 = p.whole ? p.qb : 0u;
  p.tk_done = (p.whole && p.qb > kGatherDirectBlocks) ? p.nchunks * p.nshares + p.fblocks : 0u;
  return p;
}

enum class LaunchB : uint32_t {
  kFused,
  kTwoStreams,
  kTransposed,
  kScanThenFilter,
  kPlain,
};

struct LaunchBPlan {
  LaunchB form;
  bool throughput;
  bool node_words;
  uint32_t tiles2_min;
  uint32_t nseg, share_b, scan_nsub, scan_blocks, fblocks;
  uint32_t filter_waves;
  uint32_t fused_grid;
  uint32_t launches;
};

constexpr LaunchBPlan launch_b_plan(const StepIn& in, bool fused_fits = true) {
  LaunchBPlan p{};
  const uint32_t k_est = geom_min(in.P, in.kinfo_pending ? geom_max(2u * in.h_K, 1024u) : geom_max(in.h_K, 1u));
  const uint32_t tiles = cdiv(k_est, 64u), ftiles = cdiv(2u * k_est, 64u);
  p.throughput = tiles > 16u;
  p.node_words = in.run_filter && p.throughput && in.tp_filter >= 5u && !in.no_nodew && in.have_nodew;
  p.tiles2_min = in.tp_tmin * geom_max(1u, in.nranks);
  p.nseg = in.scan_share ? in.scan_share : 8u;
  p.share_b = in.tp_share ? in.tp_share : (p.throughput ? 2u : 64u);
  p.filter_waves = in.filter_waves;
  if (p.throughput && in.tp_filter >= 5u && !in.filter_waves_env)
    p.filter_waves = in.tp_fwaves ? in.tp_fwaves
                                  : ((uint64_t)ftiles * geom_max(1u, cdiv(in.W, 2u)) >= 65536u ? geom_max(in.filter_waves, 16384u) : in.filter_waves);
  p.fblocks = in.run_filter ? filter_blocks(p.filter_waves, ftiles, in.W) : 0u;
  const uint32_t items4 = tiles * geom_min(p.nseg, cdiv(in.M, 64u)), items1 = cdiv(tiles * geom_min(p.share_b, cdiv(in.M, 64u)), 4u);
  const uint32_t cap = cdiv(in.target_waves, 4u);
  p.fused_grid = geom_max(1u, geom_min(cap, items4)) + p.fblocks + cdiv(in.P, 256u);
  const bool fused = tiles <= 16u && !in.no_fuse_final && fused_fits;
  p.scan_nsub = fused ? 4u : 1u;
  p.scan_blocks = geom_max(1u, geom_min(cap, fused ? items4 : items1));
  const bool split = p.fblocks && p.throughput;
  p.form = fused                                          ? LaunchB::kFused
           : (in.tp_filter == 8u && split)                ? LaunchB::kTwoStreams
           : (in.tp_filter >= 6u && split && in.S <= 4u)  ? LaunchB::kTransposed
           : (in.tp_filter && split)                      ? LaunchB::kScanThenFilter
                                                          : LaunchB::kPlain;
  p.launches = fused ? 2u : ((p.form == LaunchB::kTwoStreams || p.form == LaunchB::kScanThenFilter) ? 4u : 3u);
  return p;
}

}
```

### batch-scheduler_amd/csrc/bsched.hip

```cpp
#include <dlfcn.h>
#include <hip/hip_runtime.h>

#include <algorithm>
#include <cstdio>
#include <cstdlib>
#include <cstring>
#include <new>
#include <string>
#include <vector>

#ifndef BS_UNITY
#define BS_TU_MAIN
#endif
#include "bs_ctx.hpp"
#include "bs_fast.hpp"
#include "bs_epoch.hpp"
#include "bs_sort.hpp"
#include "bs_fit.hpp"
#include "bs_queue.hpp"
#include "bs_fdeny.hpp"
#include "bs_launch.hpp"
#ifdef BS_UNITY
#include "tu_fast.hip"
#include "tu_seq.hip"
// ... 650 lines not shown
                     c->d_alloc.as<int64_t>(), c->d_nreq.as<int64_t>(), c->d_rpres.as<uint32_t>(), c->d_nflags.as<uint8_t>(), c->d_left4.as<int64_t>(),
                     c->d_lglob.as<int64_t>());
}
void mirror_node_requests(bs_ctx* c, const bs_node_request* records, uint32_t n) {
  for (uint32_t i = 0; i < n; ++i) {
    const bs_node_request& r = records[i];
    for (uint32_t j = 0; j < c->L; ++j) c->h_nreq[(size_t)j * c->N + r.index] = r.requested[j];
    c->h_rpres[r.index] = r.requested_present;
  }
}

int settle_pending(bs_ctx* c) { return (c->fd_active || c->spec_active) ? fd_settle(c) : BS_OK; }
int begin_reload(bs_ctx* c) {
  int rc = use_device(c);
  if (rc) return rc;
  if ((rc = settle_pending(c))) return rc;
  c->steady_prev = -1;
  return BS_OK;
}

int check_handover(bs_ctx* c) {
  if (c->h_info.p && hinfo_get(c, kHiIdOverflow)) {
    hinfo_set(c, kHiIdOverflow, 0);
    c->pairs_ready = false;
    c->dirs_ready = false;
    c->rep_valid = false;
    c->ids_used = c->pair_cap;
    const int rc2 = derive_pods(c, false);
    c->n_rederives++;
    c->batch_void = true;
    c->last_error = "bs_pods_apply: class / pair id space overflowed on the device; the queue was re-derived, run the batch again";
    return rc2 ? rc2 : BS_ERR_RETRY;
  }
  if (c->h_info.p && hinfo_get(c, kHiHandoverErr)) {
    hinfo_set(c, kHiHandoverErr, 0);
    c->no_fuse_final = 1;
    c->batch_void = true;
    c->last_error = "in-launch hand-over timed out (producer blocks not resident): batch void, run it again (the context now uses separate launches)";
    return BS_ERR_RETRY;
  }
  if (c->batch_void) {
    c->last_error = "the last batch's results are void (hand-over time-out or queue re-derivation, reported earlier): run the batch again";
    return BS_ERR_RETRY;
  }
  return BS_OK;
}

}

extern "C" {

uint32_t bs_abi_version(void) { return BS_ABI_VERSION; }

const char* bs_strerror(int status) {
  switch (status) {
    case BS_OK: return "ok";
    case BS_ERR_INVALID: return "invalid argument";
    case BS_ERR_NO_DEVICE: return "no usable gfx950 device";
    case BS_ERR_HIP: return "HIP runtime error";
    case BS_ERR_STATE: return "call order: snapshot / groups / pods not loaded";
    case BS_ERR_CAPACITY: return "capacity exceeded";
    case BS_ERR_NOMEM: return "out of memory";
    case BS_ERR_COMM: return "RCCL error";
    case BS_ERR_RETRY: return "the last batch's results are void and the cause is repaired: run the batch again";
    default: return "unknown status";
  }
}

const char* bs_last_error(const bs_ctx* ctx) { return ctx ? ctx->last_error.c_str() : ""; }
const char* bs_kernel_name(uint32_t id) { return id < BS_KERNEL_COUNT ? kKernelNames[id] : "?"; }

static void read_env_switches(bs_ctx* c) {
  if (const char* e = std::getenv("BS_STAMP_START")) c->stamp_ctr = (uint32_t)(std::strtoul(e, nullptr, 0) % 65535u);
  if (const char* e = std::getenv("BS_KEYSEQ_START")) { c->key_seq = (uint32_t)std::strtoul(e, nullptr, 0); if (c->key_seq == 0u || c->key_seq == 0xFFFFFFFFu) c->key_seq = 1; }
  if (const char* e = std::getenv("BS_NO_FAST")) c->no_fast = std::atoi(e) ? 1u : 0u;
  if (const char* e = std::getenv("BS_NO_EPOCH")) c->no_epoch = std::atoi(e) ? 1u : 0u;
  if (const char* e = std::getenv("BS_NO_FUSE_FILTER")) c->no_fuse_filter = std::atoi(e) ? 1u : 0u;
  if (const char* e = std::getenv("BS_NO_FUSE_FINAL")) c->no_fuse_final = std::atoi(e) ? 1u : 0u;
  if (const char* e = std::getenv("BS_TP_FILTER")) c->tp_filter = (uint32_t)std::min(8, std::max(0, std::atoi(e)));
  if (const char* e = std::getenv("BS_TEST_HANDOVER_TIMEOUT")) c->test_timeout_after = (uint32_t)std::atoi(e);
  if (const char* e = std::getenv("BS_TEST_PC_CHUNK_NODES")) c->test_pc_chunk_nodes = (uint32_t)std::max(0, std::atoi(e));
  if (const char* e = std::getenv("BS_STEP_A")) { c->step_a_on = std::atoi(e) != 0; c->step_a_form = (uint32_t)std::atoi(e); }
  if (const char* e = std::getenv("BS_POD_RANGES")) c->pod_ranges_on = std::atoi(e) != 0;
  if (const char* e = std::getenv("BS_STEP_SHARES")) c->step_shares = (uint32_t)std::min(32, std::max(1, std::atoi(e)));
  if (const char* e = std::getenv("BS_TP_SHARE")) c->tp_share = (uint32_t)std::min(64, std::max(1, std::atoi(e)));
  if (const char* e = std::getenv("BS_TP_FWAVES")) c->tp_fwaves = (uint32_t)std::max(1, std::atoi(e));
  if (const char* e = std::getenv("BS_TP_SPLIT")) c->tp_split = (uint32_t)std::max(1, std::atoi(e));
  if (const char* e = std::getenv("BS_NO_NODEW")) c->no_nodew = std::atoi(e) != 0;
  if (const char* e = std::getenv("BS_TP_TMIN")) c->tp_tmin = (uint32_t)std::max(1, std::atoi(e));
  if (const char* e = std::getenv("BS_NO_SPECULATE")) c->no_spec = std::atoi(e) ? 1u : 0u;
  if (const char* e = std::getenv("BS_HOST_PROBE")) c->host_probe = std::atoi(e) ? 1u : 0u;
  if (const char* e = std::getenv("BS_HASH_SLOT_BITS")) { const int hb = std::atoi(e); c->slot_keep = hb >= 32 ? 0xFFFFFFFFu : ((1u << std::max(0, hb)) - 1u); }
  if (const char* e = std::getenv("BS_HASH_BITS")) { const int hb = std::atoi(e); c->hash_keep = hb >= 31 ? 0x7FFFFFFFu : ((1u << std::max(0, hb)) - 1u); }
  if (const char* e = std::getenv("BS_EARLY_FILTER_MIN")) { c->early_filter_min = std::strtoull(e, nullptr, 10); c->early_forced = 1; }
  if (const char* e = std::getenv("BS_SCAN_SHARE")) c->scan_share_override = (uint32_t)std::max(0, std::atoi(e));
  if (const char* e = std::getenv("BS_TARGET_WAVES")) { c->target_waves = std::max(1, std::atoi(e)); c->general_waves = c->target_waves; }
  if (const char* e = std::getenv("BS_FILTER_WAVES")) { c->filter_waves = std::max(1, std::atoi(e)); c->filter_waves_env = true; }
  if (const char* e = std::getenv("BS_SERIAL_INSERT_MAX")) c->serial_insert_max = (uint32_t)std::max(0, std::atoi(e));
  if (const char* e = std::getenv("BS_ID_ROOM")) c->id_room = (uint32_t)std::max(1, std::atoi(e));
}

int bs_create(const bs_config* cfg, bs_ctx** out) {
  if (!cfg || !out) return BS_ERR_INVALID;
  *out = nullptr;
  if (cfg->abi_version != BS_ABI_VERSION || cfg->scalar_lanes > BS_MAX_SCALARS) return BS_ERR_INVALID;
  int ndev = 0;
  if (hipGetDeviceCount(&ndev) != hipSuccess || ndev <= 0 || cfg->device < 0 || cfg->device >= ndev) return BS_ERR_NO_DEVICE;
  hipDeviceProp_t prop;
  if (hipGetDeviceProperties(&prop, cfg->device) != hipSuccess) return BS_ERR_NO_DEVICE;
  if (std::strncmp(prop.gcnArchName, "gfx950", 6) != 0) return BS_ERR_NO_DEVICE;
  bs_ctx* c = new (std::nothrow) bs_ctx();
  if (!c) return BS_ERR_NOMEM;
  c->cfg = *cfg;
  c->S = cfg->scalar_lanes;
  c->L = BS_FIXED_LANES + c->S;
  c->LP = c->S == 0 ? 4 : (c->S <= 4 ? 8 : 16);
  if (hipSetDevice(cfg->device) != hipSuccess || hipStreamCreateWithFlags(&c->stream.h, hipStreamNonBlocking) != hipSuccess ||
      hipStreamCreateWithFlags(&c->stream3.h, hipStreamNonBlocking) != hipSuccess ||
      hipEventCreateWithFlags(&c->ev_query.h, hipEventDisableTiming) != hipSuccess ||
      hipEventCreateWithFlags(&c->ev_filter.h, hipEventDisableTiming) != hipSuccess) {
    delete c;
    return BS_ERR_NO_DEVICE;
  }
  if (c->d_nepochs.reserve(64) != hipSuccess || hipMemset(c->d_nepochs.p, 0, 64) != hipSuccess || c->d_ticket.reserve(kTkWords * 4) != hipSuccess ||
      hipMemset(c->d_ticket.p, 0, kTkWords * 4) != hipSuccess) {
    delete c;
    return BS_ERR_NOMEM;
  }
  if (c->d_info.reserve(64) != hipSuccess || c->d_first_reach.reserve(64) != hipSuccess || hipMemset(c->d_first_reach.p, 0xFF, 64) != hipSuccess ||
      c->h_info.reserve(64) != hipSuccess) {
    delete c;
    return BS_ERR_NOMEM;
  }
  std::memset(c->h_info.p, 0, 64);
  c->batch_seq = 1;
  read_env_switches(c);
  *out = c;
  return BS_OK;
}

int bs_destroy(bs_ctx* c) {
  if (!c) return BS_OK;
  if (c->host_probe && c->hp_n)
    std::fprintf(stderr, "[bs host probe] %llu fast-chain batches: to chain choice %.2f us | to launch A %.2f | launch A call %.2f | to launch B %.2f | launch B call %.2f | rest %.2f\n",
                 (unsigned long long)c->hp_n, c->hp_ns[0] / 1e3 / c->hp_n, c->hp_ns[1] / 1e3 / c->hp_n, c->hp_ns[2] / 1e3 / c->hp_n, c->hp_ns[3] / 1e3 / c->hp_n,
                 c->hp_ns[4] / 1e3 / c->hp_n, c->hp_ns[5] / 1e3 / c->hp_n);
  (void)hipSetDevice(c->cfg.device);
  (void)hipStreamSynchronize(c->stream);
  (void)hipStreamSynchronize(c->stream3);
  for (auto& e : c->events) { (void)hipEventDestroy(e.a); (void)hipEventDestroy(e.b); }
  if (c->comm && c->rccl_destroy) (void)c->rccl_destroy((ncclComm_t)c->comm);
  delete c;
  return BS_OK;
}

int bs_nodes_load(bs_ctx* c, const bs_nodes_soa* nodes) {
  if (c) c->seq_wait_valid = false;
  if (!c || !nodes) return BS_ERR_INVALID;
  int rc = begin_reload(c);
  if (rc) return rc;
  const uint32_t N = nodes->n, L = c->L;
  if (N && (!nodes->allocatable || !nodes->requested || !nodes->allocatable_present || !nodes->requested_present || !nodes->flags))
    return BS_ERR_INVALID;
  if (N > 0x7FFFFFF0u) return BS_ERR_CAPACITY;
  c->N = N;
  c->h_alloc.assign(nodes->allocatable, nodes->allocatable + (size_t)L * N);
// ... 670 lines not shown
    HIPCHK(c, c->d_fu_bitmap.reserve((size_t)(cdiv(c->N, 64) + 1) * filter_cap * 8));
    HIPCHK(c, c->d_uparams.reserve((size_t)filter_cap * 64));
    if ((rc = reserve_filled(c, c->d_uflags, (size_t)filter_cap * 4, 0))) return rc;
    if ((rc = reserve_filled(c, c->d_uclaim, (size_t)filter_cap * 4, 0))) return rc;
    HIPCHK(c, c->d_nodew.reserve(nodew_alloc_words(c->N) * 8));
  }
  c->scan_slots_cap = scan_cap;
  c->filter_slots_cap = filter_cap;
  return BS_OK;
}

static int ensure_hout(bs_ctx* c) {
  const uint32_t hs = std::min<uint32_t>(c->filter_slots_cap, 1024u);
  const size_t off_feas = align256(c->olay.bytes), off_tag = off_feas + align256((size_t)hs * 4), need = off_tag + 256;
  const size_t need_rows = (size_t)(cdiv(c->N, 64) + 1) * hs * 8;
  if (need > c->h_hout.cap) {
    HIPCHK(c, c->h_hout.reserve(need));
    std::memset(c->h_hout.p, 0, need);
  }
  HIPCHK(c, c->h_hrows.reserve(need_rows));
  c->hstride = hs;
  c->off_hfeas = off_feas;
  c->off_htag = off_tag;
  return BS_OK;
}

static int setup_host_out(bs_ctx* c, uint32_t stages, bool run_filter, BatchDev& b, BatchParams& prm) {
  const bool host_out = (stages & BS_BATCH_HOST_RESULTS) && c->nranks == 1 && !c->reduce_external && !c->ext_admit && !(stages & BS_BATCH_COMMIT);
  c->last_host_out = host_out;
  if (!host_out) return BS_OK;
  int rc = ensure_hout(c);
  if (rc) return rc;
  c->host_tag = c->host_tag == 0x7FFFFFFF ? 1 : c->host_tag + 1;
  prm.host_tag = c->host_tag;
  uint8_t* h = c->h_hout.p;
  b.h_pf_code = c->olay.pf_code.in(h);
  b.h_pf_first_k = c->olay.pf_first_k.in(h);
  b.h_pf_leader = c->olay.pf_leader.in(h);
  b.h_fl_code = c->olay.fl_code.in(h);
  b.h_fl_feasible = c->olay.fl_feasible.in(h);
  b.h_fl_slot = c->olay.fl_slot.in(h);
  b.h_admit = c->olay.admit.in(h);
  b.h_ready = c->olay.ready.in(h);
  b.h_feas = reinterpret_cast<uint32_t*>(h + c->off_hfeas);
  b.h_tag = reinterpret_cast<int32_t*>(h + c->off_htag);
  b.h_rows = run_filter ? c->h_hrows.p : nullptr;
  b.hstride = c->hstride;
  return BS_OK;
}

static bool fd_commit_gated(const bs_ctx* c) {
  return c->fd_on && (hinfo_get(c, kHiFdFound) || hinfo_get(c, kHiFdChanged));
}
static bool handover_commit_gated(const bs_ctx* c) {
  return c->h_info.p && hinfo_get(c, kHiHandoverErr) != 0;
}

static int launch_filter_deny(bs_ctx* c, const PodsDev& pd, const GroupsDev& gr, const NodesDev& nd, const BatchDev& b, BatchParams prm, bool tail) {
  if (!c->P) return BS_OK;
  prm.seq_inv = ~c->key_seq;
  c->fd_seq_inv = prm.seq_inv;
  const dim3 grid(cdiv(c->P, 256)), blk(256);
  TIMED(c, BS_KERNEL_RESOLVE, {
    if (!tail) hipLaunchKernelGGL(k_fd_events, grid, blk, 0, c->stream, pd, gr, nd, b, prm);
    hipLaunchKernelGGL(k_fd_apply, grid, blk, 0, c->stream, pd, gr, nd, b, prm, tail ? 1u : 0u);
  });
  c->launches += tail ? 1 : 2;
  return BS_OK;
}
static int launch_filter_deny_marks(bs_ctx* c, const BatchDev& b, BatchParams prm, uint32_t* reject) {
  if (!c->G) return BS_OK;
  prm.seq_inv = c->fd_seq_inv;
  hipLaunchKernelGGL(k_fd_reject, dim3(cdiv(c->G, 256)), dim3(256), 0, c->stream, b, prm, reject, c->G);
  LAUNCHCHK(c, BS_KERNEL_RESOLVE);
  c->launches++;
  return BS_OK;
}

static inline uint64_t host_ns() {
  timespec ts;
  clock_gettime(CLOCK_MONOTONIC, &ts);
  return (uint64_t)ts.tv_sec * 1000000000ull + (uint64_t)ts.tv_nsec;
}
static int step_a_residency(bs_ctx* c, bool whole) {
  int& r = c->step_a_resident[whole ? 1 : 0];
  if (r < 0) r = step_a_residency_query(fast_launch(c), whole);
  return r;
}

static BatchParams chain_params(const bs_ctx* c, uint32_t stages, bool use_classes, bool stamped = true) {
  BatchParams prm = batch_params(c);
  prm.run_filter = (stages & BS_STAGE_FILTER) ? 1u : 0u;
  prm.use_classes = use_classes ? 1u : 0u;
  prm.fuse_filter = prm.run_filter;
  prm.scan_slots_cap = c->scan_slots_cap;
  prm.filter_slots_cap = c->filter_slots_cap;
  if (!stamped) return prm;
  prm.stamp = 1u + c->stamp_ctr;
  prm.seq_inv = ~c->key_seq;
  prm.do_tally = (stages & BS_STAGE_TALLY) ? 1u : 0u;
  prm.do_ready = (prm.do_tally && c->nranks == 1 && !c->reduce_external) ? 1u : 0u;
  return prm;
}

static BatchDev table_view(const bs_ctx* c, const BatchDev& b, const BatchParams& prm, uint32_t slot) {
  BatchDev bt = b;
  bt.tables = b.tables + (size_t)slot * prm.mcap * prm.LP;
  bt.kp = b.kp + (size_t)slot * 16;
  bt.chunk_tot = b.chunk_tot + (size_t)slot * cdiv(c->Ncap, 256) * 16;
  bt.chunk_kp = b.chunk_kp + (size_t)slot * cdiv(c->Ncap, 256) * 16;
  bt.gmax = b.gmax + (size_t)slot * cdiv(c->Ncap, 64) * prm.LP;
  return bt;
}

static StepIn step_in(const bs_ctx* c, bool run_filter) {
  StepIn in{};
  in.P = c->P; in.G = c->G; in.N = c->N; in.M = c->M; in.S = c->S; in.W = cdiv(c->N, 64);
  in.kinfo_pending = c->kinfo_pending; in.h_K = c->h_K; in.k_bound = c->k_bound; in.k_host = c->kinfo_pending ? 0u : c->h_K;
  in.step_a_form = c->step_a_form; in.step_a_on = c->step_a_on; in.step_shares = c->step_shares;
  in.filter_waves = c->filter_waves; in.filter_waves_env = c->filter_waves_env;
  in.tp_filter = c->tp_filter; in.tp_share = c->tp_share; in.tp_fwaves = c->tp_fwaves; in.tp_tmin = c->tp_tmin;
  in.target_waves = c->target_waves; in.scan_share = c->scan_share_override; in.nranks = c->nranks;
  in.run_filter = run_filter; in.dirs_ready = c->dirs_ready;
  in.ranges_valid = c->ranges_valid && c->d_pod_ranges.p; in.nranges = c->nranges;
  in.whole_bufs = c->d_first_row64.p && c->d_scan_rec.p && c->d_feas_rec.p && c->d_chunk_rec.p;
  in.no_fuse_final = c->no_fuse_final; in.no_nodew = c->no_nodew; in.have_nodew = c->d_nodew.p != nullptr;
  in.collect_stats = c->collect_stats; in.enable_timing = c->cfg.enable_timing;
  return in;
}

static int fast_commit_tail(bs_ctx* c, uint32_t stages, const PodsDev& pd, const GroupsDev& gr, const NodesDev& nd, const BatchDev& b, const BatchParams& prm) {
  int rc;
  const uint32_t P = c->P, G = c->G;
  if (prm.filter_deny && (rc = launch_filter_deny(c, pd, gr, nd, b, prm, true))) return rc;
  if (prm.commit) {
    if (prm.filter_deny && (rc = launch_filter_deny_marks(c, b, prm, b.fast_reject))) return rc;
    if (G) hipLaunchKernelGGL(k_fast_commit, dim3(cdiv(G, 256)), dim3(256), 0, c->stream, pd, b, const_cast<uint8_t*>(gr.flags),
                              const_cast<uint64_t*>(gr.occupied), G, prm.filter_deny ? b.fd_flag : nullptr);
    LAUNCHCHK(c, BS_KERNEL_RESOLVE);
    int32_t last = -1;
    HIPCHK(c, hipMemcpyAsync(&last, b.pf_leader + (P - 1), 4, hipMemcpyDeviceToHost, c->stream));
    if (G) HIPCHK(c, hipMemcpyAsync(c->h_gflags.data(), gr.flags, G, hipMemcpyDeviceToHost, c->stream));
    HIPCHK(c, hipStreamSynchronize(c->stream));
    if (!fd_commit_gated(c) && !handover_commit_gated(c)) c->sop_leader0 = last;
    c->launches++;
  }
  return batch_collective(c, stages, gr, b);
}

static int launch_b(bs_ctx* c, const LaunchBPlan& pl, const FastLaunch& fl, const PodsDev& pd, const GroupsDev& gr, const NodesDev& nd, const BatchDev& b,
                    const BatchDev& bt, const BatchParams& prm) {
  switch (pl.form) {
    case LaunchB::kFused:
      launch_fast_bc(fl, dim3(pl.fused_grid), pd, gr, nd, b, bt, prm, pl.nseg, pl.scan_blocks, pl.fblocks);
      break;
    case LaunchB::kTwoStreams: {
      FastLaunch side = fl;
      side.stream = c->stream3;
      HIPCHK(c, hipEventRecord(c->ev_query, c->stream));
      HIPCHK(c, hipStreamWaitEvent(c->stream3, c->ev_query, 0));
      launch_fast_scan(side, dim3(pl.scan_blocks), bt, prm, pl.share_b);
      HIPCHK(c, hipEventRecord(c->ev_filter, c->stream3));
      launch_fast_filter(fl, dim3(pl.fblocks), pd, nd, bt, prm);
      HIPCHK(c, hipStreamWaitEvent(c->stream, c->ev_filter, 0));
      break;
    }
    case LaunchB::kTransposed:
      launch_fast_bt(fl, dim3(pl.scan_blocks + pl.fblocks), nd, bt, prm, pl.share_b, pl.scan_blocks);
      break;
    case LaunchB::kScanThenFilter:
      launch_fast_scan(fl, dim3(pl.scan_blocks), bt, prm, pl.share_b);
      launch_fast_filter(fl, dim3(pl.fblocks), pd, nd, bt, prm);
      break;
    case LaunchB::kPlain:
      launch_fast_b(fl, dim3(pl.scan_blocks + pl.fblocks), pd, nd, bt, prm, pl.share_b, pl.scan_blocks);
      break;
  }
  return BS_OK;
}

static int run_fast(bs_ctx* c, uint32_t stages) {
  int rc;
  const uint32_t P = c->P, G = c->G, N = c->N;
  const bool run_filter = stages & BS_STAGE_FILTER;
  NodesDev nd = nodes_dev(c);
  GroupsDev gr = groups_dev(c);
  PodsDev pd = pods_dev(c);
  BatchDev b = batch_dev(c);
  BatchParams prm = chain_params(c, stages, true);
  prm.commit = (stages & BS_BATCH_COMMIT) ? 1u : 0u;
  if ((rc = setup_host_out(c, stages, run_filter, b, prm))) return rc;
  const uint32_t side_slot = (uint32_t)c->steady_table;
  const uint32_t nchunks = table_chunks(c->M);
  BatchDev bt = table_view(c, b, prm, side_slot);
  const TableDesc* forced = b.desc + side_slot;
  if (prm.commit && G) HIPCHK(c, hipMemsetAsync(c->d_fast_reject.p, 0xFF, (size_t)G * 4, c->stream));

  if (c->kinfo_pending && hinfo_get(c, kHiKTag) == c->kinfo_tag && (rc = resolve_pods(c))) return rc;
  StepIn in = step_in(c, run_filter);
  prm.k_host = in.k_host;
  const uint64_t hp1 = c->host_probe ? host_ns() : 0;
  const uint32_t K = step_k(in);
  const bool dirs_buildable = c->batch_since_pods && c->pairs_ready && c->rep_valid && c->have_groups;
  if (step_a_possible(in, K, nchunks) && (c->step_a_form == 1u || c->dirs_ready || dirs_buildable)) {
    if (c->step_a_form >= 2u && !c->dirs_ready && dirs_buildable && (rc = build_dirs(c))) return rc;
    in.dirs_ready = c->dirs_ready;
    const StepAPlan pa = step_a_plan(in, K);
    if (pa.ranges) b.pod_ranges = c->d_pod_ranges.as<uint32_t>();
    if (pa.ready && (int)pa.grid <= step_a_residency(c, pa.whole)) {
      TIMED(c, BS_KERNEL_QUERY, {
        launch_fast_step_a(fast_launch(c), dim3(pa.grid), pd, gr, nd, b, bt, prm, forced, pa.nchunks, pa.qb, pa.nshares, pa.fblocks, c->tk_pods, c->tk_tab, pa.pb,
                           c->d_ckeys.as<int64_t>(), c->d_cpres.as<uint32_t>(), c->pair_cap, pa.whole ? 1u : 0u, c->tk_p1, c->tk_done, side_slot - c->C);
      });
      c->tk_pods += pa.tk_pods;
      c->tk_tab += pa.tk_tab;
      c->tk_p1 += pa.tk_p1;
      c->tk_done += pa.tk_done;
      if (!pa.whole) TIMED(c, BS_KERNEL_RESOLVE, hipLaunchKernelGGL(k_fast_final, dim3(cdiv(P, 256)), dim3(256), 0, c->stream, pd, gr, nd, b, prm, cdiv(P, kTblChunk)));
      c->launches = pa.launches;
      c->last_step_a = true;
      if (c->test_timeout_after && --c->test_timeout_after == 0 && c->h_info.p) {
        HIPCHK(c, hipStreamSynchronize(c->stream));
        hinfo_set(c, kHiHandoverErr, 1);
      }
      return fast_commit_tail(c, stages, pd, gr, nd, b, prm);
    }
  }
  c->last_step_a = false;
  LaunchBPlan pl = launch_b_plan(in);
  if (pl.node_words) {
    b.nodew = bt.nodew = c->d_nodew.as<uint64_t>();
    b.nodew_stride = bt.nodew_stride = nodew_stride(N);
    b.tiles2_min = bt.tiles2_min = pl.tiles2_min;
  }
  TIMED(c, BS_KERNEL_QUERY, {
    const uint32_t qb = cdiv(P, kTblChunk);
    const dim3 qg(qb + nchunks + (pl.node_words ? nodew_blocks(N) : 0u)), blk(kTblChunk);
    lanes_narrow(c->S, [&](auto s) {
      hipLaunchKernelGGL(HIP_KERNEL_NAME(k_fast_query_tables<decltype(s)::value>), qg, blk, 0, c->stream, pd, gr, nd, b, bt, prm, forced, nchunks, qb);
    });
  });
  const uint64_t hp2 = c->host_probe ? host_ns() : 0;
  uint64_t hp3 = 0;
  TIMED(c, BS_KERNEL_SCAN, {
    if (pl.form == LaunchB::kFused && (int)pl.fused_grid > fused_residency(c)) pl = launch_b_plan(in, false);
    prm.scan_nsub = pl.scan_nsub;
    hp3 = c->host_probe ? host_ns() : 0;
    if ((rc = launch_b(c, pl, fast_launch(c, pl.filter_waves), pd, gr, nd, b, bt, prm))) return rc;
  });
  if (c->host_probe) {
    const uint64_t hp4 = host_ns();
    c->hp_ns[0] += c->hp_t1 - c->hp_t0; c->hp_ns[1] += hp1 - c->hp_t1; c->hp_ns[2] += hp2 - hp1; c->hp_ns[3] += hp3 - hp2; c->hp_ns[4] += hp4 - hp3;
    c->hp_n++;
  }
  if (pl.form != LaunchB::kFused) TIMED(c, BS_KERNEL_RESOLVE, hipLaunchKernelGGL(k_fast_final, dim3(cdiv(P, 256)), dim3(256), 0, c->stream, pd, gr, nd, b, prm, cdiv(P, kTblChunk)));
  c->launches = pl.launches;
  return fast_commit_tail(c, stages, pd, gr, nd, b, prm);
}

static int commit_readback(bs_ctx* c, const GroupsDev& gr, const BatchDev& b) {
  const uint32_t P = c->P, G = c->G;
  std::vector<uint32_t> cls(G);
  if (P) {
    int32_t last = -1;
    HIPCHK(c, hipMemcpyAsync(&last, b.pf_leader + (P - 1), 4, hipMemcpyDeviceToHost, c->stream));
    HIPCHK(c, hipStreamSynchronize(c->stream));
    if (fd_commit_gated(c)) return BS_OK;
    c->sop_leader0 = last;
  }
  if (G) {
    HIPCHK(c, hipMemcpy(c->h_gflags.data(), gr.flags, G, hipMemcpyDeviceToHost));
    HIPCHK(c, hipMemcpy(cls.data(), gr.cls, (size_t)G * 4, hipMemcpyDeviceToHost));
  }
  c->n_uncaptured = 0;
  c->n_nominres = 0;
  c->max_group_cls = 0;
  for (uint32_t i = 0; i < G; ++i) {
    if (!(c->h_gflags[i] & BS_GROUP_HAS_POD)) c->n_uncaptured++;
    else c->max_group_cls = std::max(c->max_group_cls, cls[i]);
    if (!(c->h_gflags[i] & BS_GROUP_HAS_MINRES)) c->n_nominres++;
  }
  return BS_OK;
}

static int run_epoch(bs_ctx* c, uint32_t stages, bool* taken) {
  int rc;
  *taken = false;
  if (!c->epochs_ready && (rc = analyse_epochs(c))) return rc;
  if ((rc = resolve_pods(c)) || (rc = resolve_epochs(c))) return rc;
  const uint32_t P = c->P, G = c->G, N = c->N, C = c->C, K = c->h_K, R = c->h_R;
  const uint32_t W = cdiv(N, 64);
  const bool run_filter = stages & BS_STAGE_FILTER;
  if ((c->h_eflags & 4u) || R == 0 || R > kMaxRuns || K == 0) return BS_OK;
  const uint32_t GB = cdiv(2 * R * K, 64) * 64;
  const uint32_t filter_slots = (R + 1) * K;
  if ((uint64_t)GB + G > c->scan_slots_cap || filter_slots > c->filter_slots_cap || filter_slots > P) return BS_OK;
  *taken = true;
  NodesDev nd = nodes_dev(c);
  GroupsDev gr = groups_dev(c);
  PodsDev pd = pods_dev(c);
  BatchDev b = batch_dev(c);
  BatchParams prm = chain_params(c, stages, false);
  EpochDev ep{};
  ep.run_of_epoch = c->d_run_of_epoch.as<uint32_t>();
  ep.run_leader = c->d_run_leader.as<int32_t>();
  ep.gslot = c->d_gslot.as<uint32_t>();
  ep.gfirstq = c->d_gfirstq.as<unsigned long long>();
  ep.R = R; ep.K = K; ep.GB = GB;
  ep.has_first = c->h_eflags & 1u;
  ep.has_reserve = (c->h_eflags >> 1) & 1u;
  if ((rc = setup_host_out(c, stages, run_filter, b, prm))) return rc;
// ... 279 lines not shown
  }
}

static int fd_resolve(bs_ctx* c) {
  if (!c->fd_active) return BS_OK;
  c->fd_active = false;
  c->fd_unsynced = false;
  if (!hinfo_get(c, kHiFdFound)) return BS_OK;
  int rc = BS_OK;
  bool settled = false;
  const uint32_t stages = c->fd_stages;
  for (uint32_t iter = 1; iter <= c->P + 2 && !settled; ++iter) {
    BatchDev b = batch_dev(c);
    b.fd_in = c->d_fd_in.as<uint32_t>();
    BatchParams prm = batch_params(c);
    prm.seq_inv = c->fd_seq_inv;
    hipLaunchKernelGGL(k_fd_next, dim3(cdiv(std::max<uint32_t>(c->G, 1), 256)), dim3(256), 0, c->stream, b, prm, c->G);
    LAUNCHCHK(c, BS_KERNEL_RESOLVE);
    c->fd_in_live = true;
    c->fd_iter = iter;
    c->epochs_ready = false;
    discard_handover(c);
    rc = batch_run_inner(c, stages);
    if (rc == BS_OK) rc = hipStreamSynchronize(c->stream) == hipSuccess ? BS_OK : BS_ERR_HIP;
    c->n_fd_reruns++;
    if (rc) break;
    settled = !hinfo_get(c, kHiFdChanged);
  }
  c->fd_in_live = false;
  c->fd_iter = 0;
  c->fd_on = false;
  c->epochs_ready = false;
  if (rc) return rc;
  if (!settled) { c->last_error = "BS_BATCH_FILTER_DENY: the fixed-point iteration did not settle"; return BS_ERR_STATE; }
  return BS_OK;
}

static int fd_settle(bs_ctx* c) {
  if (!c->fd_active && !c->spec_active) return BS_OK;
  if (!c->batch_since_pods) { c->fd_active = false; c->spec_active = false; return BS_OK; }
  int rc;
  if (c->last_host_out) {
    if ((rc = wait_host_tag(c, 0, c->host_tag, reinterpret_cast<const int32_t*>(c->h_hout.p + c->off_htag)))) return rc;
  } else {
    HIPCHK(c, hipStreamSynchronize(c->stream));
  }
  if (c->spec_active) {
    c->spec_active = false;
    if ((rc = resolve_groups(c))) return rc;
    if (c->steady_table != c->spec_table) {
      c->n_spec_miss++;
      const bool fd = c->fd_active;
      discard_handover(c);
      if ((rc = batch_run_inner(c, c->spec_stages))) return rc;
      c->fd_active = fd;
      HIPCHK(c, hipStreamSynchronize(c->stream));
    }
  }
  return fd_resolve(c);
}

int bs_batch_run(bs_ctx* c, uint32_t stages) {
  if (!c) return BS_ERR_INVALID;
  if (!c->have_nodes || !c->have_fit || !c->have_groups || !c->have_pods) {
    c->last_error = "bs_batch_run needs nodes, fit, groups and pods loaded";
    return BS_ERR_STATE;
  }
  if (!(stages & BS_STAGE_PREFILTER)) { c->last_error = "PREFILTER stage is mandatory"; return BS_ERR_INVALID; }
  if ((stages & BS_BATCH_COMMIT) && c->nranks > 1) { c->last_error = "COMMIT is single-rank only"; return BS_ERR_STATE; }
  if (stages & BS_BATCH_FILTER_DENY) {
    if (!(stages & BS_STAGE_FILTER)) { c->last_error = "BS_BATCH_FILTER_DENY needs BS_STAGE_FILTER"; return BS_ERR_INVALID; }
    if (c->nranks > 1 || c->reduce_external) { c->last_error = "BS_BATCH_FILTER_DENY is single-rank only"; return BS_ERR_STATE; }
  }
  int rc = use_device(c);
  if (rc) return rc;
  if ((stages & BS_BATCH_FILTER_DENY) && c->fd_unsynced) {
    HIPCHK(c, hipStreamSynchronize(c->stream));
    c->fd_unsynced = false;
  }
  c->fd_active = false;
  c->fd_iter = 0;
  c->fd_in_live = false;
  c->batch_void = false;
  rc = batch_run_inner(c, stages);
  if (rc == BS_OK && (stages & BS_BATCH_FILTER_DENY) && c->P) c->fd_unsynced = true;
  if (rc == BS_OK && (stages & BS_BATCH_FILTER_DENY) && c->P) {
    c->fd_active = true;
    c->fd_stages = stages;
    if (stages & BS_BATCH_COMMIT) {
      HIPCHK(c, hipStreamSynchronize(c->stream));
      rc = fd_resolve(c);
    }
  }
  return rc;
}

int bs_batch_finish(bs_ctx* c) {
  if (!c) return BS_ERR_INVALID;
  if (!c->have_groups) return BS_ERR_STATE;
  int rc = use_device(c);
  if (rc) return rc;
  if (c->G) hipLaunchKernelGGL(k_ready, dim3(cdiv(c->G, 256)), dim3(256), 0, c->stream, groups_dev(c), batch_dev(c));
  HIPCHK(c, hipGetLastError());
  c->batch_pending_finish = false;
  return BS_OK;
}

int bs_batch_sync(bs_ctx* c) {
  if (!c) return BS_ERR_INVALID;
  int rc = use_device(c);
  if (rc) return rc;
  if ((rc = fd_settle(c))) return rc;
  HIPCHK(c, hipStreamSynchronize(c->stream));
  c->h_dstage.busy = false;
  return check_handover(c);
}

static int filter_rows_of(bs_ctx* c, uint32_t* rows) {
  int rc = resolve_pods(c);
  if (rc) return rc;
  const bool classes = c->batch_since_pods ? c->last_use_classes : (c->n_uncaptured == 0 && c->n_nominres == 0);
  *rows = c->P ? (classes ? 2 * c->h_K : c->P) : 0;
  if (c->batch_since_pods && c->last_chain == 2) *rows = c->last_rows;
  return BS_OK;
}

int bs_filter_rows_count(bs_ctx* c, uint32_t* rows) {
  if (!c || !rows) return BS_ERR_INVALID;
  if (!c->have_pods || !c->have_groups) return BS_ERR_STATE;
  int rc = use_device(c);
  if (rc) return rc;
  return filter_rows_of(c, rows);
}

int bs_batch_read(bs_ctx* c, const bs_batch_out* out) {
  if (!c || !out) return BS_ERR_INVALID;
  if (!c->have_pods || !c->have_groups) return BS_ERR_STATE;
  int rc = use_device(c);
  if (rc) return rc;
  if ((rc = fd_settle(c))) return rc;
  const uint32_t P = c->P, G = c->G, W = cdiv(c->N, 64);
  const bool filtered = c->last_stages & BS_STAGE_FILTER;
  const bool want_pod = P && (out->pf_code || out->pf_first_k || out->pf_leader || out->fl_code || out->fl_feasible || out->fl_slot);
  const bool want_grp = G && (c->last_stages & BS_STAGE_TALLY) && (out->group_admit || out->group_ready);
  auto copy_out = [&](const uint8_t* st, const void* admit) {
    if (want_pod) {
      if (out->pf_code) std::memcpy(out->pf_code, c->olay.pf_code.in(st), P);
      if (out->pf_first_k) std::memcpy(out->pf_first_k, c->olay.pf_first_k.in(st), (size_t)P * 4);
      if (out->pf_leader) std::memcpy(out->pf_leader, c->olay.pf_leader.in(st), (size_t)P * 4);
      if (out->fl_code) std::memcpy(out->fl_code, c->olay.fl_code.in(st), P);
      if (out->fl_feasible) std::memcpy(out->fl_feasible, c->olay.fl_feasible.in(st), (size_t)P * 4);
      if (out->fl_slot) std::memcpy(out->fl_slot, c->olay.fl_slot.in(st), (size_t)P * 4);
    }
    if (want_grp) {
      if (out->group_admit) std::memcpy(out->group_admit, admit, (size_t)G * 4);
      if (out->group_ready) std::memcpy(out->group_ready, c->olay.ready.in(st), G);
    }
  };
  uint32_t nrows = 0;
  if (out->fl_rows || out->fl_rows_feasible || out->fl_rows_n) {
    if (filtered && (rc = filter_rows_of(c, &nrows))) return rc;
    if (out->fl_rows_n) *out->fl_rows_n = nrows;
    if ((out->fl_rows || out->fl_rows_feasible) && nrows > out->fl_rows_cap) {
      c->last_error = "bs_batch_read: fl_rows_cap is smaller than the rows of the batch";
      return BS_ERR_CAPACITY;
    }
// ... 499 lines not shown
  if (!h) h = dlopen("librccl.so.1", RTLD_NOW | RTLD_LOCAL);
  if (!h) h = dlopen("librccl.so", RTLD_NOW | RTLD_LOCAL);
  return h;
}

int bs_comm_unique_id(uint8_t id[128]) {
  if (!id) return BS_ERR_INVALID;
  static_assert(sizeof(ncclUniqueId) == 128, "the ABI hands the RCCL unique id over as 128 bytes");
  void* h = open_rccl();
  if (!h) return BS_ERR_COMM;
  auto f = (decltype(&ncclGetUniqueId))dlsym(h, "ncclGetUniqueId");
  ncclUniqueId u;
  if (!f || f(&u) != ncclSuccess) return BS_ERR_COMM;
  std::memcpy(id, u.internal, 128);
  return BS_OK;
}

int bs_comm_init(bs_ctx* c, const uint8_t id[128], uint32_t rank, uint32_t nranks) {
  if (!c || !id || nranks == 0 || rank >= nranks) return BS_ERR_INVALID;
  int rc = use_device(c);
  if (rc) return rc;
  void* h = open_rccl();
  if (!h) { c->last_error = std::string("dlopen librccl: ") + (dlerror() ? dlerror() : "?"); return BS_ERR_COMM; }
  ncclUniqueId u;
  std::memcpy(u.internal, id, 128);
  auto init = (decltype(&ncclCommInitRank))dlsym(h, "ncclCommInitRank");
  c->rccl_allreduce = (decltype(&ncclAllReduce))dlsym(h, "ncclAllReduce");
  c->rccl_destroy = (decltype(&ncclCommDestroy))dlsym(h, "ncclCommDestroy");
  ncclComm_t comm = nullptr;
  if (!init || !c->rccl_allreduce || !c->rccl_destroy) { c->last_error = "librccl lacks ncclCommInitRank / ncclAllReduce / ncclCommDestroy"; return BS_ERR_COMM; }
  const ncclResult_t r = init(&comm, (int)nranks, u, (int)rank);
  if (r != ncclSuccess) { c->last_error = std::string("ncclCommInitRank failed: code ") + std::to_string((int)r); return BS_ERR_COMM; }
  c->rccl_handle = h;
  c->comm = comm;
  c->rank = rank;
  c->nranks = nranks;
  return BS_OK;
}

#ifdef BS_PROBE
int bs_probe_read(bs_ctx* c, unsigned long long* out) {
  if (!c || !out) return BS_ERR_INVALID;
  int rc = use_device(c);
  if (rc) return rc;
  HIPCHK(c, hipStreamSynchronize(c->stream));
  HIPCHK(c, hipMemcpyFromSymbol(out, HIP_SYMBOL(g_probe), sizeof(g_probe)));
  static std::vector<unsigned long long> zero(sizeof(g_probe) / 8, 0ull);
  HIPCHK(c, hipMemcpyToSymbol(HIP_SYMBOL(g_probe), zero.data(), sizeof(g_probe)));
  return BS_OK;
}
#endif

int bs_timing_reset(bs_ctx* c) {
  if (!c) return BS_ERR_INVALID;
  int rc = use_device(c);
  if (rc) return rc;
  rc = timer_collect(c);
  std::memset(&c->timing, 0, sizeof(c->timing));
  return rc;
}

int bs_timing_get(bs_ctx* c, bs_timing* out) {
  if (!c || !out) return BS_ERR_INVALID;
  int rc = use_device(c);
  if (rc) return rc;
  rc = timer_collect(c);
  *out = c->timing;
  return rc;
}

int bs_speculation_stats(const bs_ctx* c, uint64_t* launched, uint64_t* missed) {
  if (!c || !launched || !missed) return BS_ERR_INVALID;
  *launched = c->n_spec;
  *missed = c->n_spec_miss;
  return BS_OK;
}

int bs_filter_deny_stats(const bs_ctx* c, uint64_t* reruns) {
  if (!c || !reruns) return BS_ERR_INVALID;
  *reruns = c->n_fd_reruns;
  return BS_OK;
}

int bs_batch_stats_get(bs_ctx* c, bs_batch_stats* out) {
  if (!c || !out) return BS_ERR_INVALID;
  int rc = use_device(c);
  if (rc) return rc;
  std::memset(out, 0, sizeof(*out));
  if (!c->collect_stats) {
    c->collect_stats = 1;
    return BS_OK;
  }
  HIPCHK(c, hipStreamSynchronize(c->stream));
  uint64_t raw[8] = {0};
  uint32_t nt = 0, nq = 0;
  if (c->d_stats.p) HIPCHK(c, hipMemcpy(raw, c->d_stats.p, sizeof(raw), hipMemcpyDeviceToHost));
  if (c->d_qcount.p) HIPCHK(c, hipMemcpy(&nq, c->d_qcount.p, 4, hipMemcpyDeviceToHost));
  if (c->d_needed.p && c->C) {
    std::vector<uint32_t> need(2 * c->C);
    HIPCHK(c, hipMemcpy(need.data(), c->d_needed.p, need.size() * 4, hipMemcpyDeviceToHost));
    for (uint32_t x : need) nt += x ? 1u : 0u;
  }
  out->scan_rows_executed = raw[0];
  out->scan_evals_executed = raw[1];
  out->scan_queries = raw[4];
  out->scan_queries_logical = raw[2];
  out->filter_lane_blocks = raw[5];
  out->filter_tile_blocks = raw[6];
  out->class_mode = c->last_use_classes ? 1 : 0;
  out->fast_path = c->last_fast ? 1 : 0;
  out->chain = c->last_chain;
  out->launches = c->launches;
  out->tables_built = c->last_fast ? 1 : nt;
  out->logical_evals = (uint64_t)c->P * c->N;
  out->filter_evals = (c->last_stages & BS_STAGE_FILTER) ? (uint64_t)c->P * c->N : 0;
  if (c->last_stages & BS_STAGE_FILTER) {
    out->filter_distinct = raw[3];
    out->filter_evals_executed = raw[3] * c->N;
  }
  c->collect_stats = 0;
  return BS_OK;
}

}
```

### batch-scheduler_amd/csrc/tu_fast.hip

```cpp
#ifndef BS_UNITY
#define BS_TU_FAST
#endif
#include "bs_fast.hpp"
#include "bs_launch.hpp"

#include <algorithm>

namespace bs {

void launch_fast_b(const FastLaunch& c, dim3 grid, const PodsDev& pd, const NodesDev& nd, const BatchDev& bt, const BatchParams& prm, uint32_t nseg,
                          uint32_t scan_blocks) {
  lanes_wide(c.S, [&](auto s) {
    hipLaunchKernelGGL(HIP_KERNEL_NAME(k_fast_scan_filter<decltype(s)::value>), grid, dim3(256), 0, c.stream, pd, nd, bt, prm, c.M, nseg, scan_blocks,
                       c.filter_waves, c.filter_slots_cap);
  });
}
void launch_fast_scan(const FastLaunch& c, dim3 grid, const BatchDev& bt, const BatchParams& prm, uint32_t nseg) {
  lanes_wide(c.S, [&](auto s) { hipLaunchKernelGGL(HIP_KERNEL_NAME(k_fast_scan<decltype(s)::value>), grid, dim3(256), 0, c.stream, bt, prm, c.M, nseg); });
}
void launch_fast_bt(const FastLaunch& c, dim3 grid, const NodesDev& nd, const BatchDev& bt, const BatchParams& prm, uint32_t nseg, uint32_t scan_blocks) {
  lanes_clamped(c.S, [&](auto s) {
    hipLaunchKernelGGL(HIP_KERNEL_NAME(k_fast_scan_filter_t<decltype(s)::value>), grid, dim3(256), 0, c.stream, nd, bt, prm, c.M, nseg, scan_blocks,
                       c.filter_split ? c.filter_split : c.filter_waves, c.filter_slots_cap, (c.tp_filter == 7u ? 1u : 0u) | (c.filter_split ? 2u : 0u));
  });
}
void launch_fast_filter(const FastLaunch& c, dim3 grid, const PodsDev& pd, const NodesDev& nd, const BatchDev& bt, const BatchParams& prm) {
  switch (c.tp_filter) {
    case 1: hipLaunchKernelGGL(HIP_KERNEL_NAME(k_fast_filter<4, true>), grid, dim3(256), 0, c.stream, pd, nd, bt, prm, c.filter_waves, c.filter_slots_cap); break;
    case 2: hipLaunchKernelGGL(HIP_KERNEL_NAME(k_fast_filter<2, true>), grid, dim3(256), 0, c.stream, pd, nd, bt, prm, c.filter_waves, c.filter_slots_cap); break;
    case 3: hipLaunchKernelGGL(HIP_KERNEL_NAME(k_fast_filter<2, false>), grid, dim3(256), 0, c.stream, pd, nd, bt, prm, c.filter_waves, c.filter_slots_cap); break;
    case 4: hipLaunchKernelGGL(k_fast_filter_w7, grid, dim3(256), 0, c.stream, pd, nd, bt, prm, c.filter_waves, c.filter_slots_cap); break;
    default: hipLaunchKernelGGL(k_fast_filter_t, grid, dim3(256), 0, c.stream, nd, bt, prm, c.filter_split ? c.filter_split : c.filter_waves, c.filter_slots_cap, c.filter_split ? 1u : 0u); break;
  }
}
template <class K>
static int blocks_resident(const FastLaunch& c, K kernel, int block) {
  int per_cu = 0;
  if (hipOccupancyMaxActiveBlocksPerMultiprocessor(&per_cu, kernel, block, 0) != hipSuccess || per_cu <= 0) return 0;
  hipDeviceProp_t prop;
  if (hipGetDeviceProperties(&prop, c.device) != hipSuccess) return 0;
  return std::max(0, per_cu - 1) * prop.multiProcessorCount;
}
int fused_residency_query(const FastLaunch& c) {
  return lanes_wide(c.S, [&](auto s) { return blocks_resident(c, k_fast_scan_filter_final<decltype(s)::value>, 256); });
}
void launch_fast_bc(const FastLaunch& c, dim3 grid, const PodsDev& pd, const GroupsDev& gr, const NodesDev& nd, const BatchDev& b, const BatchDev& bt,
                           const BatchParams& prm, uint32_t nseg, uint32_t scan_blocks, uint32_t filter_blocks) {
  lanes_wide(c.S, [&](auto s) {
    hipLaunchKernelGGL(HIP_KERNEL_NAME(k_fast_scan_filter_final<decltype(s)::value>), grid, dim3(256), 0, c.stream, pd, gr, nd, b, bt, prm, c.M, nseg,
                       scan_blocks, filter_blocks, c.filter_waves, c.filter_slots_cap, cdiv(c.P, kTblChunk));
  });
}

void launch_fast_step_a(const FastLaunch& c, dim3 grid, const PodsDev& pd, const GroupsDev& gr, const NodesDev& nd, const BatchDev& b, const BatchDev& bt,
                        const BatchParams& prm, const TableDesc* forced, uint32_t nchunks, uint32_t query_blocks, uint32_t nshares, uint32_t filter_blocks,
                        uint32_t tk_pods0, uint32_t tk_tab0, uint32_t param_blocks, const int64_t* ckeys, const uint32_t* cpres, uint32_t kcap,
                        uint32_t whole, uint32_t tk_p1, uint32_t tk_done, uint32_t forced_cls) {
  lanes_clamped(c.S, [&](auto s) {
    auto launch = [&](auto whole_step) {
      hipLaunchKernelGGL(HIP_KERNEL_NAME(k_fast_step_a<decltype(s)::value, decltype(whole_step)::value>), grid, dim3(kTblChunk), 0, c.stream, pd, gr, nd, b, bt,
                         prm, forced, nchunks, query_blocks, nshares, filter_blocks, c.filter_waves, c.filter_slots_cap, tk_pods0, tk_tab0, param_blocks,
                         ckeys, cpres, kcap, tk_p1, tk_done, forced_cls);
    };
    if (whole) launch(std::true_type{});
    else launch(std::false_type{});
  });
}
int step_a_residency_query(const FastLaunch& c, bool whole) {
  return lanes_clamped(c.S, [&](auto s) {
    constexpr int TS = decltype(s)::value;
    return whole ? blocks_resident(c, k_fast_step_a<TS, true>, (int)kTblChunk) : blocks_resident(c, k_fast_step_a<TS, false>, (int)kTblChunk);
  });
}

}
```

### include/bsched.h

```cpp
#ifndef BSCHED_H
#define BSCHED_H

#include <stddef.h>
#include <stdint.h>

#ifdef __cplusplus
extern "C" {
#endif

#define BS_ABI_VERSION 7u

enum {
  BS_LANE_CPU = 0,
  BS_LANE_MEM = 1,
  BS_LANE_EPH = 2,
  BS_LANE_PODS = 3,
  BS_FIXED_LANES = 4,
  BS_MAX_SCALARS = 12,
  BS_MAX_LANES = 16
};

typedef enum bs_status {
  BS_OK = 0,
  BS_ERR_INVALID = -1,
// ... 467 lines not shown
int bs_batch_read_flat(bs_ctx* ctx, uint8_t* pf_code, uint32_t* pf_first_k, int32_t* pf_leader, uint8_t* fl_code, uint32_t* fl_feasible,
                       uint64_t* fl_bitmap, uint32_t* group_admit, uint8_t* group_ready, uint32_t* fl_slot, uint64_t* fl_rows,
                       uint32_t* fl_rows_feasible, uint32_t fl_rows_cap, uint32_t* fl_rows_n);
int bs_seq_run_flat(bs_ctx* ctx, uint32_t stages, uint8_t* pf_code, uint32_t* pf_first_k, int32_t* pf_leader, int32_t* pod_node, uint32_t cap,
                    uint32_t* released_group, uint32_t* released_pods, int64_t* first_ns, int64_t* ready_ns, int64_t* scalars_out,
                    uint8_t* last_permitted);
int bs_seq_run_nominated_flat(bs_ctx* ctx, uint32_t stages, uint32_t p, const int32_t* priority, const uint32_t* own_id, uint8_t* pf_code,
                              uint32_t* pf_first_k, int32_t* pf_leader, int32_t* pod_node, uint32_t cap, uint32_t* released_group,
                              uint32_t* released_pods, int64_t* first_ns, int64_t* ready_ns, int64_t* scalars_out, uint8_t* last_permitted);
int bs_seq_run_scored_flat(bs_ctx* ctx, uint32_t stages, uint32_t w_least, uint32_t w_most, uint32_t w_balanced, uint8_t* pf_code,
                           uint32_t* pf_first_k, int32_t* pf_leader, int32_t* pod_node, uint32_t cap, uint32_t* released_group,
                           uint32_t* released_pods, int64_t* first_ns, int64_t* ready_ns, int64_t* scalars_out, uint8_t* last_permitted);
int bs_seq_run_scored_nominated_flat(bs_ctx* ctx, uint32_t stages, uint32_t p, const int32_t* priority, const uint32_t* own_id, uint32_t w_least,
                                     uint32_t w_most, uint32_t w_balanced, uint8_t* pf_code, uint32_t* pf_first_k, int32_t* pf_leader, int32_t* pod_node,
                                     uint32_t cap, uint32_t* released_group, uint32_t* released_pods, int64_t* first_ns, int64_t* ready_ns,
                                     int64_t* scalars_out, uint8_t* last_permitted);
int bs_fit_build_flat(bs_ctx* ctx, uint32_t n, const uint32_t* name, const uint32_t* label_off, const uint32_t* label_key, const uint32_t* label_val,
                      const int64_t* label_int, const uint8_t* label_int_ok, const uint32_t* taint_off, const uint32_t* taint_key,
                      const uint32_t* taint_val, const uint8_t* taint_effect,
                      uint32_t c, uint32_t field_name_key, const uint8_t* tpl_flags, const uint32_t* sel_off, const uint32_t* sel_key,
                      const uint32_t* sel_val, const uint32_t* term_off, const uint32_t* term_expr_off, const uint32_t* term_field_off,
                      uint32_t ex_count, const uint32_t* ex_key, const uint8_t* ex_op, const uint32_t* ex_val_off, const uint32_t* ex_val,
                      const int64_t* ex_val_int, const uint8_t* ex_val_int_ok,
                      uint32_t fd_count, const uint32_t* fd_key, const uint8_t* fd_op, const uint32_t* fd_val_off, const uint32_t* fd_val,
                      const int64_t* fd_val_int, const uint8_t* fd_val_int_ok,
                      const uint32_t* tol_off, const uint32_t* tol_key, const uint32_t* tol_val, const uint8_t* tol_op, const uint8_t* tol_effect);

int bs_bound_load_flat(bs_ctx* ctx, uint32_t b, const uint32_t* node, const int32_t* priority, const int64_t* start_ns, const int32_t* group,
                       const int64_t* req, const uint32_t* req_present);
int bs_preempt_run_flat(bs_ctx* ctx, uint32_t stages, uint32_t count, const uint32_t* pod_index, const int32_t* priority, const uint8_t* group_protected,
                        uint32_t victim_cap, int32_t* node, uint32_t* n_candidates, uint32_t* n_victims, uint32_t* victims, int32_t* top_priority,
                        int64_t* priority_sum, int64_t* earliest_start);
int bs_bound_apply_flat(bs_ctx* ctx, uint32_t n_remove, const uint32_t* remove, uint32_t n_insert, const uint32_t* node, const int32_t* priority,
                        const int64_t* start_ns, const int32_t* group, const int64_t* req, const uint32_t* req_present,
                        const uint8_t* pdb_violating, uint32_t* first_id_out);
int bs_bound_apply_ex_flat(bs_ctx* ctx, uint32_t flags, uint32_t n_remove, const uint32_t* remove, uint32_t n_insert, const uint32_t* node,
                           const int32_t* priority, const int64_t* start_ns, const int32_t* group, const int64_t* req,
                           const uint32_t* req_present, const uint8_t* pdb_violating, uint32_t* first_id_out);
int bs_preempt_commit_flat(bs_ctx* ctx, uint32_t stages, uint32_t count, const uint32_t* pod_index, const int32_t* priority,
                           const uint8_t* group_protected, uint32_t flags, uint32_t victim_cap, int32_t* node, uint32_t* n_candidates,
                           uint32_t* n_victims, uint32_t* victims, int32_t* top_priority, int64_t* priority_sum, int64_t* earliest_start);
int bs_seq_expire_flat(bs_ctx* ctx, uint32_t count, const uint32_t* group, uint32_t flags, uint32_t group_cap, uint32_t* group_out,
                       uint32_t* group_pods, uint32_t* group_earlier, uint32_t pod_cap, uint32_t* pod, uint32_t* node, uint32_t* counts_out );
int bs_preempt_commit_gang_flat(bs_ctx* ctx, uint32_t stages, uint32_t count, const uint32_t* pod_index, const int32_t* priority,
                                const uint8_t* group_protected, const uint32_t* gang_need, uint32_t flags, uint32_t victim_cap,
                                int32_t* node, uint32_t* n_candidates, uint32_t* n_victims, uint32_t* victims, int32_t* top_priority,
                                int64_t* priority_sum, int64_t* earliest_start);
int bs_groups_list_apply_flat(bs_ctx* ctx, uint32_t n_remove, const uint32_t* remove, uint32_t n_update, const uint32_t* update, uint32_t rows_g,
                              const uint32_t* min_member, const uint32_t* status_scheduled, const uint32_t* matched, const uint8_t* flags,
                              const uint32_t* cls, const int64_t* min_resources, const uint32_t* min_resources_present, const uint64_t* occupied_by,
                              uint32_t n_append, uint32_t wait_cap, uint32_t* wait_id, uint32_t* wait_node, int32_t* wait_group,
                              uint32_t* counts_out );

#define BS_KERNEL_PREPASS   0u
#define BS_KERNEL_LEADER    1u
#define BS_KERNEL_QUERY     2u
#define BS_KERNEL_TABLES    3u
#define BS_KERNEL_SCAN      4u
#define BS_KERNEL_RESOLVE   5u
#define BS_KERNEL_FILTER    6u
#define BS_KERNEL_TALLY     7u
#define BS_KERNEL_COUNT     8u
typedef struct bs_timing {
  double   total_ms[BS_KERNEL_COUNT];
  uint64_t launches[BS_KERNEL_COUNT];
} bs_timing;
int bs_timing_reset(bs_ctx* ctx);
int bs_timing_get(bs_ctx* ctx, bs_timing* out);
const char* bs_kernel_name(uint32_t kernel_id);
typedef struct bs_batch_stats {
  uint64_t scan_queries, scan_rows_executed, scan_evals_executed, tables_built, logical_evals;
  uint64_t filter_evals;
  uint64_t filter_distinct;
  uint64_t filter_evals_executed;
  uint64_t scan_queries_logical;
  uint64_t class_mode;
  uint64_t fast_path;
  uint64_t launches;
  uint64_t chain;
  uint64_t filter_lane_blocks;
  uint64_t filter_tile_blocks;
} bs_batch_stats;
int bs_batch_stats_get(bs_ctx* ctx, bs_batch_stats* out);
int bs_pods_apply_stats(const bs_ctx* ctx, uint64_t* applies, uint64_t* rederives);
int bs_filter_deny_stats(const bs_ctx* ctx, uint64_t* reruns);
int bs_speculation_stats(const bs_ctx* ctx, uint64_t* launched, uint64_t* missed);

#ifdef __cplusplus
}
#endif
#endif
```

Before: 3778 billion evals/s.

## Add whole-table step-A scan blocks that cover all nodes in register strips

Adds a table_whole_block path in the fused step-A kernel: each block scans every node in per-wave strips held in registers, using a small prefetch ring of row loads, and resolves all of its class queries against those prefix sums. The usual chunk×share grid of table-scan blocks is replaced by one block per share, placed after the filter blocks, which is meant to remove cross-chunk combining and atomics on the first-row results. Strip-count template variants are dispatched on node count, and the host falls back to the old form if residency or the plan does not allow it. The trade-offs are higher register pressure (waves_per_eu hint), serial per-query ballots over strips, and an error flag when the per-share class count exceeds the cap. A step_form query API is added for introspection.

```diff
diff --git a/batch-scheduler_amd/capi.py b/batch-scheduler_amd/capi.py
--- a/batch-scheduler_amd/capi.py
+++ b/batch-scheduler_amd/capi.py
@@ -21,7 +21,7 @@
     "bs_cluster_fits", "bs_node_left", "bs_scan_prefix", "bs_cluster_total", "bs_filter_one", "bs_find_max_pg",
     "bs_batch_run", "bs_batch_sync", "bs_batch_read", "bs_batch_map", "bs_filter_rows_count", "bs_queue_order_load", "bs_queue_sort",
     "bs_shard_set", "bs_reduce_external", "bs_group_admit_devptr", "bs_group_admit_bind", "bs_stream", "bs_comm_unique_id", "bs_comm_init", "bs_batch_finish",
-    "bs_timing_reset", "bs_timing_get", "bs_kernel_name", "bs_batch_stats_get",
+    "bs_timing_reset", "bs_timing_get", "bs_kernel_name", "bs_batch_stats_get", "bs_step_form_get",
     "bs_seq_run", "bs_nodes_read", "bs_first_reach_hint",
     "bs_nodes_load_flat", "bs_groups_load_flat", "bs_groups_read_flat", "bs_pods_load_flat", "bs_pods_apply_flat", "bs_pods_read_flat",
     "bs_batch_read_flat", "bs_seq_run_flat", "bs_fit_build_flat",
@@ -212,6 +212,7 @@
     L.bs_timing_reset.argtypes = [vp]
     L.bs_timing_get.argtypes = [vp, P(Timing)]
     L.bs_batch_stats_get.argtypes = [vp, P(BatchStats)]
+    L.bs_step_form_get.argtypes = [vp, P(u32)]
     L.bs_seq_run.argtypes = [vp, u32, P(SeqOut)]
     L.bs_nodes_read.argtypes = [vp, P(C.c_int64), P(u32)]
     L.bs_bound_load.argtypes = [vp, P(soa.BoundStruct)]
@@ -1103,6 +1104,11 @@
         self._chk(self._lib.bs_timing_get(self._h, C.byref(t)), "bs_timing_get")
         return {self._lib.bs_kernel_name(i).decode(): (float(t.total_ms[i]), int(t.launches[i])) for i in range(KERNEL_COUNT)}
 
+    def step_form(self) -> dict:
+        f = (C.c_uint32 * 4)()
+        self._chk(self._lib.bs_step_form_get(self._h, f), "bs_step_form_get")
+        return {"whole_step": bool(f[0]), "table_whole": bool(f[1]), "table_blocks": int(f[2]), "filter_blocks": int(f[3])}
+
     def stats_arm(self):
         s = BatchStats()
         self._chk(self._lib.bs_batch_stats_get(self._h, C.byref(s)), "bs_batch_stats_get")
diff --git a/batch-scheduler_amd/csrc/bs_ctx.hpp b/batch-scheduler_amd/csrc/bs_ctx.hpp
--- a/batch-scheduler_amd/csrc/bs_ctx.hpp
+++ b/batch-scheduler_amd/csrc/bs_ctx.hpp
@@ -234,6 +234,7 @@
   uint32_t tp_split = 0;
   int fused_blocks_resident = -1;
   int step_a_resident[2] = {-1, -1};
+  int step_a_resident_tw[3] = {-1, -1, -1};
   uint32_t step_a_form = 3;
   bool step_a_on = true;
   uint32_t step_shares = 8;
@@ -248,6 +249,8 @@
   std::vector<uint32_t> h_pod_ranges;
   DevBuf d_pod_ranges;
   bool last_step_a = false;
+  bool step_table_whole = true;
+  uint32_t step_form[4] = {0, 0, 0, 0};
   uint32_t scan_share_override = 0, no_fuse_filter = 0, early_forced = 0, target_waves = 8192, filter_waves = 8192, collect_stats = 0;
   uint32_t general_waves = 4096;
   bs_batch_stats stats{};
diff --git a/batch-scheduler_amd/csrc/bs_fast.hpp b/batch-scheduler_amd/csrc/bs_fast.hpp
--- a/batch-scheduler_amd/csrc/bs_fast.hpp
+++ b/batch-scheduler_amd/csrc/bs_fast.hpp
@@ -572,6 +572,33 @@
     if (++spins > kSpinBound) { if (h_err && lane_id() == 0) __hip_atomic_store(h_err, 1, __ATOMIC_RELAXED, __HIP_MEMORY_SCOPE_SYSTEM); return false; }
   }
 }
+struct TableRow {
+  uint32_t fw, ap, rp;
+  uint8_t fl;
+  int64_t al[BS_MAX_LANES], rq[BS_MAX_LANES];
+};
+__device__ __forceinline__ void table_row_load(const NodesDev& nd, const TableDesc& d, uint32_t L, uint32_t n, TableRow& r) {
+  r.fw = nd.fit[(size_t)d.cls * nd.fit_words + (n >> 5)];
+  r.fl = nd.flags[n];
+  r.ap = nd.apres[n];
+  r.rp = nd.rpres[n];
+#pragma unroll
+  for (uint32_t j = 0; j < BS_MAX_LANES; ++j) {
+    if (j < L) {
+      r.al[j] = nd.alloc[(size_t)j * nd.stride + n];
+      r.rq[j] = nd.req[(size_t)j * nd.stride + n];
+    }
+  }
+}
+template <bool NODES>
+__device__ __forceinline__ bool table_row_valid(const TableRow& r, bool in_range) { return in_range && (!NODES || !(r.fl & BS_NODE_SKIP_MASK)); }
+__device__ __forceinline__ bool table_row_fit(const TableRow& r, bool valid, uint32_t n) { return valid && ((r.fw >> (n & 31u)) & 1u) && !(r.fl & BS_NODE_TAINT_ERR); }
+__device__ __forceinline__ uint32_t table_row_pres(const TableRow& r, bool fit) { return fit ? (r.ap & r.rp) : 0u; }
+__device__ __forceinline__ unsigned long long table_row_left(const TableRow& r, const TableDesc& d, const BatchParams& prm, bool fit, uint32_t pres, uint32_t j) {
+  const bool live = fit && (j < 4 || (pres & (1u << (j - 4)))) && !(j == BS_LANE_EPH && !prm.eph_gate);
+  return live ? (unsigned long long)wsub(scale_f32(r.al[j], d.pct), r.rq[j]) : 0ull;
+}
+
 template <int TS, bool REGS = false>
 __device__ __forceinline__ void table_scan_block(const NodesDev& nd, const BatchDev& b, const BatchParams& prm, const TableDesc* forced, uint32_t chunk, uint32_t nchunks,
                                                  uint32_t share, uint32_t nshares, uint32_t pod_blocks, uint32_t tk_pods0, uint32_t tk_tab0, const GroupsDev& gr,
@@ -590,18 +617,9 @@
   const bool in_range = REGS ? k < nd.n : k < nd.m;
   const uint32_t n = REGS ? (in_range ? k : 0u) : (in_range ? nd.kmap[k] : 0u);
   const TableDesc d = REGS ? TableDesc{forced_cls, 0.7f} : *forced;
-  const uint32_t fw = nd.fit[(size_t)d.cls * nd.fit_words + (n >> 5)];
-  const uint8_t fl = nd.flags[n];
-  const bool valid = in_range && (!REGS || !(fl & BS_NODE_SKIP_MASK));
-  const uint32_t ap = nd.apres[n], rp = nd.rpres[n];
-  int64_t al[BS_MAX_LANES], rq[BS_MAX_LANES];
-#pragma unroll
-  for (uint32_t j = 0; j < BS_MAX_LANES; ++j) {
-    if (j < L) {
-      al[j] = nd.alloc[(size_t)j * nd.stride + n];
-      rq[j] = nd.req[(size_t)j * nd.stride + n];
-    }
-  }
+  TableRow tr;
+  table_row_load(nd, d, L, n, tr);
+  const bool valid = table_row_valid<REGS>(tr, in_range);
   const uint32_t K = prm.k_host ? prm.k_host : *b.kclass;
   const uint32_t per = (K + nshares - 1u) / nshares, s_lo = share * per, s_hi = min(K, s_lo + per);
   Res raw;
@@ -618,8 +636,8 @@
     panic0 = b.panic_epoch[0];
     if (gr.g) leader_pre_load(gr, leader0, sh, lp0);
   }
-  const bool fit = valid && ((fw >> (n & 31u)) & 1u) && !(fl & BS_NODE_TAINT_ERR);
-  const uint32_t pres = fit ? (ap & rp) : 0u;
+  const bool fit = table_row_fit(tr, valid, n);
+  const uint32_t pres = table_row_pres(tr, fit);
   if (threadIdx.x < BS_MAX_SCALARS) s_kp[threadIdx.x] = BS_INF;
   for (uint32_t t = threadIdx.x; t < kStepSlotsMax; t += kTblChunk) s_first[t] = BS_INF;
   unsigned long long incl[BS_MAX_LANES];
@@ -628,9 +646,7 @@
   for (uint32_t j = 0; j < BS_MAX_LANES; ++j) {
     incl[j] = 0;
     if (j < L) {
-      const bool live = fit && (j < 4 || (pres & (1u << (j - 4)))) && !(j == BS_LANE_EPH && !prm.eph_gate);
-      const unsigned long long left = live ? (unsigned long long)wsub(scale_f32(al[j], d.pct), rq[j]) : 0ull;
-      incl[j] = wave_incl_scan_add_u64(left);
+      incl[j] = wave_incl_scan_add_u64(table_row_left(tr, d, prm, fit, pres, j));
       if (lane_id() == 63) s_wtot[j][w] = incl[j];
     }
   }
@@ -844,6 +860,173 @@
   for (uint32_t t = threadIdx.x; t < nmine; t += kTblChunk) {
     if (s_first[t] == BS_INF) continue;
     atomicMin(&b.first_row[s_lo + t], s_first[t]);
+  }
+  BS_STAMP(2, 7);
+}
+
+template <int TS, int NS>
+__device__ __forceinline__ void table_whole_block(const NodesDev& nd, const BatchDev& b, const BatchParams& prm, uint32_t share, uint32_t nshares, const GroupsDev& gr,
+                                                  const int64_t* ckeys, const uint32_t* cpres, uint32_t kcap, bool direct, uint32_t forced_cls) {
+  __shared__ unsigned long long s_wtot[BS_MAX_LANES][4];
+  __shared__ uint32_t s_kp[BS_MAX_SCALARS];
+  __shared__ int64_t s_req[kTableWholePer][BS_MAX_LANES];
+  __shared__ uint32_t s_qf[kTableWholePer];
+  __shared__ uint32_t s_first[kTableWholePer];
+  BS_STAMP(2, 0);
+  const Shape<TS> sh(prm.S);
+  const uint32_t L = sh.L(), S = sh.S();
+  const int w = wave_id();
+  const uint32_t ns = min((nd.n + 255u) / 256u, (uint32_t)NS);
+  const uint32_t wrow = (uint32_t)__builtin_amdgcn_readfirstlane((int)((uint32_t)w * ns * 64u));
+  const uint32_t q0 = wrow + (uint32_t)lane_id();
+  const TableDesc d{forced_cls, 0.7f};
+  const uint32_t K = prm.k_host ? prm.k_host : *b.kclass;
+  const uint32_t per = (K + nshares - 1u) / nshares, s_lo = share * per, s_hi = min(K, s_lo + per);
+  const uint32_t nmine = s_hi > s_lo ? min(s_hi - s_lo, kTableWholePer) : 0u;
+  if (per > kTableWholePer && threadIdx.x == 0 && b.h_err) __hip_atomic_store(b.h_err, 1, __ATOMIC_RELAXED, __HIP_MEMORY_SCOPE_SYSTEM);
+  Res raw;
+  LeaderPre lp0{};
+  const uint32_t cc = threadIdx.x < nmine ? s_lo + threadIdx.x : 0u;
+#pragma unroll
+  for (uint32_t j = 0; j < BS_MAX_LANES; ++j)
+    if (j < L) raw.v[j] = ckeys[(size_t)j * kcap + cc];
+  raw.present = cpres[cc];
+  const int32_t leader0 = b.leader_epoch[0];
+  const uint8_t panic0 = b.panic_epoch[0];
+  if (gr.g) leader_pre_load(gr, leader0, sh, lp0);
+  if (threadIdx.x < BS_MAX_SCALARS) s_kp[threadIdx.x] = BS_INF;
+  if (threadIdx.x < kTableWholePer) s_first[threadIdx.x] = BS_INF;
+  auto derive_queries = [&]() {
+    if (threadIdx.x < nmine) {
+      uint32_t qf = 0x80000000u;
+      Res q;
+      res_zero(q, sh);
+      if (leader0 >= 0 && !panic0) {
+        Res cur;
+        res_zero(cur, sh);
+        res_add(cur, raw, sh, prm.eph_gate);
+        qf = class_scan_query(cur, lp0, sh, prm.eph_gate, q);
+      }
+      s_qf[threadIdx.x] = qf;
+#pragma unroll
+      for (uint32_t j = 0; j < BS_MAX_LANES; ++j)
+        if (j < L) s_req[threadIdx.x][j] = q.v[j];
+    }
+  };
+  constexpr int kQueryStrip = NS > 2 ? 2 : NS - 1;
+  static_assert(NS >= 1 && NS <= 32, "one validity bit per strip");
+  unsigned long long incl[NS][4 + TS], tot[4 + TS];
+  uint32_t vbits = 0;
+  uint32_t kfirst[BS_MAX_SCALARS];
+#pragma unroll
+  for (uint32_t j = 0; j < 4u + (uint32_t)TS; ++j) tot[j] = 0ull;
+#pragma unroll
+  for (uint32_t s2 = 0; s2 < BS_MAX_SCALARS; ++s2) kfirst[s2] = BS_INF;
+  constexpr int kRowRegs = 4 * (4 + TS) + 4, kRing = (200 - NS * 2 * (4 + TS)) / kRowRegs >= 4 ? 4 : (200 - NS * 2 * (4 + TS)) / kRowRegs >= 3 ? 3 : 2;
+  constexpr int kAhead = kRing - 1 < NS ? kRing - 1 : NS;
+  TableRow ring[kRing];
+  auto strip_row = [&](int i, bool& in_range) -> uint32_t {
+    const uint32_t k = q0 + (uint32_t)i * 64u;
+    in_range = (uint32_t)i < ns && k < nd.n;
+    return in_range ? k : 0u;
+  };
+#pragma unroll
+  for (int i = 0; i < kAhead; ++i) {
+    bool in_range;
+    table_row_load(nd, d, L, strip_row(i, in_range), ring[i % kRing]);
+  }
+#pragma unroll
+  for (int i = 0; i < NS; ++i) {
+    if (i + kAhead < NS) {
+      bool in_range;
+      table_row_load(nd, d, L, strip_row(i + kAhead, in_range), ring[(i + kAhead) % kRing]);
+    }
+    __builtin_amdgcn_sched_barrier(0);
+    bool in_range;
+    const uint32_t n = strip_row(i, in_range);
+    const TableRow& tr = ring[i % kRing];
+    const bool valid = table_row_valid<true>(tr, in_range);
+    const bool fit = table_row_fit(tr, valid, n);
+    const uint32_t pres = table_row_pres(tr, fit);
+    vbits |= valid ? 1u << i : 0u;
+#pragma unroll
+    for (uint32_t j = 0; j < 4u + (uint32_t)TS; ++j) {
+      incl[i][j] = wave_incl_scan_add_u64(table_row_left(tr, d, prm, fit, pres, j));
+      tot[j] += bcast64(incl[i][j], 63);
+    }
+#pragma unroll
+    for (uint32_t s2 = 0; s2 < BS_MAX_SCALARS; ++s2) {
+      if (s2 < S) {
+        const unsigned long long mk = __ballot(valid && (pres & (1u << s2)));
+        kfirst[s2] = (mk && kfirst[s2] == BS_INF) ? wrow + (uint32_t)i * 64u + (uint32_t)(__ffsll((long long)mk) - 1) : kfirst[s2];
+      }
+    }
+    if (i == kQueryStrip) derive_queries();
+  }
+  if (lane_id() == 0) {
+#pragma unroll
+    for (uint32_t j = 0; j < 4u + (uint32_t)TS; ++j) s_wtot[j][w] = tot[j];
+  }
+  __syncthreads();
+#pragma unroll
+  for (uint32_t s2 = 0; s2 < BS_MAX_SCALARS; ++s2)
+    if (s2 < S && kfirst[s2] != BS_INF && lane_id() == 0) atomicMin(&s_kp[s2], kfirst[s2]);
+  BS_STAMP(2, 1);
+  {
+    unsigned long long base[4 + TS];
+#pragma unroll
+    for (uint32_t j = 0; j < 4u + (uint32_t)TS; ++j) {
+      base[j] = 0ull;
+#pragma unroll
+      for (int i = 0; i < 4; ++i)
+        if (i < w) base[j] += s_wtot[j][i];
+    }
+#pragma unroll
+    for (int i = 0; i < NS; ++i) {
+#pragma unroll
+      for (uint32_t j = 0; j < 4u + (uint32_t)TS; ++j) {
+        const unsigned long long t = bcast64(incl[i][j], 63);
+        incl[i][j] += base[j];
+        base[j] += t;
+      }
+    }
+  }
+  __syncthreads();
+  uint32_t kpg[BS_MAX_SCALARS];
+#pragma unroll
+  for (uint32_t s2 = 0; s2 < BS_MAX_SCALARS; ++s2) kpg[s2] = s2 < S ? s_kp[s2] : BS_INF;
+  BS_STAMP(2, 3);
+  const uint32_t smask = S ? ((1u << S) - 1u) : 0u;
+  for (uint32_t t = 0; t < nmine; ++t) {
+    const uint32_t qf = s_qf[t];
+    if (qf & 0x80000000u) continue;
+    int64_t r[4 + TS];
+#pragma unroll
+    for (uint32_t j = 0; j < 4u + (uint32_t)TS; ++j) r[j] = s_req[t][j];
+    const uint32_t nab = ~(qf >> 16) & smask;
+    uint32_t best = BS_INF;
+#pragma unroll
+    for (int i = 0; i < NS; ++i) {
+      if (best == BS_INF) {
+        const uint32_t k = q0 + (uint32_t)i * 64u;
+        uint32_t keyrow = 0;
+#pragma unroll
+        for (uint32_t s2 = 0; s2 < BS_MAX_SCALARS; ++s2)
+          if (s2 < S && k >= kpg[s2]) keyrow |= 1u << s2;
+        unsigned long long m = __ballot(((vbits >> i) & 1u) && (nab & ~keyrow) == 0u);
+#pragma unroll
+        for (uint32_t j = 0; j < 4u + (uint32_t)TS; ++j) m &= __ballot((int64_t)incl[i][j] >= r[j]);
+        if (m) best = wrow + (uint32_t)i * 64u + (uint32_t)(__ffsll((long long)m) - 1);
+      }
+    }
+    if (best != BS_INF && lane_id() == 0) atomicMin(&s_first[t], best);
+  }
+  __syncthreads();
+  BS_STAMP(2, 4);
+  if (threadIdx.x < nmine) {
+    const unsigned long long word = ((unsigned long long)prm.seq_inv << 32) | s_first[threadIdx.x];
+    if (direct) st_pub<true>(&b.scan_rec[s_lo + threadIdx.x], word);
+    else if (s_first[threadIdx.x] != BS_INF) atomicMin(&b.first_row64[s_lo + threadIdx.x], word);
   }
   BS_STAMP(2, 7);
 }
@@ -1371,8 +1554,8 @@
   fast_final_block(pods, gr, nd, b, prm, query_blocks, blockIdx.x - producers, gridDim.x - producers, producers);
 }
 
-template <int TS, bool WHOLE>
-__global__ __launch_bounds__(kTblChunk) void k_fast_step_a(PodsDev pods, GroupsDev gr, NodesDev nd, BatchDev b, BatchDev bt, BatchParams prm, const TableDesc* forced,
+template <int TS, bool WHOLE, int TW = 0>
+__global__ __launch_bounds__(kTblChunk) __attribute__((amdgpu_waves_per_eu(TW ? 2 : 1))) void k_fast_step_a(PodsDev pods, GroupsDev gr, NodesDev nd, BatchDev b, BatchDev bt, BatchParams prm, const TableDesc* forced,
                                                            uint32_t nchunks, uint32_t query_blocks, uint32_t nshares, uint32_t filter_blocks, uint32_t filter_waves,
                                                            uint32_t ustride, uint32_t tk_pods0, uint32_t tk_tab0, uint32_t param_blocks, const int64_t* ckeys,
                                                            const uint32_t* cpres, uint32_t kcap, uint32_t tk_p1, uint32_t tk_done, uint32_t forced_cls) {
@@ -1381,7 +1564,8 @@
   const uint32_t tb = nchunks * nshares;
 #ifdef BS_TEST_LATE_ROLE
   {
-    const int role = blockIdx.x < query_blocks ? 0 : blockIdx.x < query_blocks + param_blocks ? 1 : blockIdx.x < query_blocks + param_blocks + tb ? 2 : 3;
+    const bool second = blockIdx.x >= query_blocks + param_blocks + (TW > 0 ? filter_blocks : tb);
+    const int role = blockIdx.x < query_blocks ? 0 : blockIdx.x < query_blocks + param_blocks ? 1 : second == (TW > 0) ? 2 : 3;
     if (role == BS_TEST_LATE_ROLE) for (int spin = 0; spin < 20; ++spin) __builtin_amdgcn_s_sleep(127);
   }
 #endif
@@ -1408,9 +1592,10 @@
     }
   } else if (blockIdx.x < query_blocks + param_blocks) {
     class_slots_block<TS>(gr, b, prm, ckeys, cpres, kcap, blockIdx.x - query_blocks, !(WHOLE && direct));
-  } else if (blockIdx.x < query_blocks + param_blocks + tb) {
-    const uint32_t x = blockIdx.x - query_blocks - param_blocks;
-    table_scan_block<TS, WHOLE>(nd, bt, prm, forced, x / nshares, nchunks, x % nshares, nshares, producers, tk_pods0, tk_tab0, gr, ckeys, cpres, kcap, direct, forced_cls);
+  } else if (TW > 0 ? blockIdx.x >= query_blocks + param_blocks + filter_blocks : blockIdx.x < query_blocks + param_blocks + tb) {
+    const uint32_t x = blockIdx.x - query_blocks - param_blocks - (TW > 0 ? filter_blocks : 0u);
+    if constexpr (WHOLE && TW > 0) table_whole_block<TS, TW>(nd, bt, prm, x, nshares, gr, ckeys, cpres, kcap, direct, forced_cls);
+    else table_scan_block<TS, WHOLE>(nd, bt, prm, forced, x / nshares, nchunks, x % nshares, nshares, producers, tk_pods0, tk_tab0, gr, ckeys, cpres, kcap, direct, forced_cls);
     if constexpr (WHOLE) {
       if (!direct) {
         asm volatile("s_waitcnt vmcnt(0)" ::: "memory");
@@ -1419,7 +1604,7 @@
       }
     }
   } else if constexpr (WHOLE) {
-    step_filter_block<TS>(gr, nd, bt, prm, ckeys, cpres, kcap, filter_waves, ustride, blockIdx.x - query_blocks - param_blocks - tb, filter_blocks, direct, tk_pods0, producers);
+    step_filter_block<TS>(gr, nd, bt, prm, ckeys, cpres, kcap, filter_waves, ustride, blockIdx.x - query_blocks - param_blocks - (TW > 0 ? 0u : tb), filter_blocks, direct, tk_pods0, producers);
     if (!direct) {
       asm volatile("s_waitcnt vmcnt(0)" ::: "memory");
       __syncthreads();
diff --git a/batch-scheduler_amd/csrc/bs_launch.hpp b/batch-scheduler_amd/csrc/bs_launch.hpp
--- a/batch-scheduler_amd/csrc/bs_launch.hpp
+++ b/batch-scheduler_amd/csrc/bs_launch.hpp
@@ -24,7 +24,7 @@
 void launch_fast_step_a(const FastLaunch& c, dim3 grid, const PodsDev& pd, const GroupsDev& gr, const NodesDev& nd, const BatchDev& b, const BatchDev& bt,
                         const BatchParams& prm, const TableDesc* forced, uint32_t nchunks, uint32_t query_blocks, uint32_t nshares, uint32_t filter_blocks,
                         uint32_t tk_pods0, uint32_t tk_tab0, uint32_t param_blocks, const int64_t* ckeys, const uint32_t* cpres, uint32_t kcap,
-                        uint32_t whole, uint32_t tk_p1, uint32_t tk_done, uint32_t forced_cls);
-int step_a_residency_query(const FastLaunch& c, bool whole);
+                        uint32_t whole, uint32_t tk_p1, uint32_t tk_done, uint32_t forced_cls, uint32_t table_strips = 0);
+int step_a_residency_query(const FastLaunch& c, bool whole, uint32_t table_strips = 0);
 
 }
diff --git a/batch-scheduler_amd/csrc/bs_step_geom.hpp b/batch-scheduler_amd/csrc/bs_step_geom.hpp
--- a/batch-scheduler_amd/csrc/bs_step_geom.hpp
+++ b/batch-scheduler_amd/csrc/bs_step_geom.hpp
@@ -37,6 +37,7 @@
   bool no_fuse_final, no_nodew, have_nodew;
   bool collect_stats;
   int enable_timing;
+  uint32_t table_whole;
 };
 
 constexpr uint32_t table_chunks(uint32_t M) { return geom_max(1u, cdiv(M, 256u)); }
@@ -50,9 +51,21 @@
          in.enable_timing < 2 && in.S <= 4;
 }
 
+constexpr uint32_t kTableWholeStrips[3] = {2u, 4u, 10u};
+constexpr uint32_t kTableWholePer = 2u;
+constexpr uint32_t table_whole_strips_max(uint32_t S) { return S <= 3u ? 10u : 4u; }
+constexpr uint32_t table_whole_n_max(uint32_t S) { return 256u * table_whole_strips_max(S); }
+constexpr bool table_whole_fits(const StepIn& in) { return in.table_whole && in.S <= 4u && in.N <= table_whole_n_max(in.S); }
+constexpr uint32_t table_whole_strips(uint32_t N) {
+  const uint32_t need = geom_max(1u, cdiv(N, 256u));
+  return need <= kTableWholeStrips[0] ? kTableWholeStrips[0] : need <= kTableWholeStrips[1] ? kTableWholeStrips[1] : need <= kTableWholeStrips[2] ? kTableWholeStrips[2] : 0u;
+}
+constexpr uint32_t table_whole_blocks(uint32_t K) { return geom_max(1u, geom_min(cdiv(K, kTableWholePer), 128u)); }
+
 struct StepAPlan {
   bool ready;
   bool whole, ranges;
+  bool table_whole;
   uint32_t qb, pb, nchunks, nshares, fblocks, grid;
   uint32_t launches;
   uint32_t tk_pods, tk_tab, tk_p1, tk_done;
@@ -66,6 +79,8 @@
   const uint32_t nch_nodes = geom_max(1u, cdiv(in.N, 256u));
   p.whole = in.step_a_form >= 3u && p.pb && nch_nodes <= 64u && in.whole_bufs;
   p.nchunks = p.whole ? nch_nodes : table_chunks(in.M);
+  p.table_whole = p.whole && table_whole_fits(in);
+  if (p.table_whole) { p.nchunks = 1u; p.nshares = table_whole_blocks(K); }
   p.ranges = p.whole && in.ranges_valid && in.nranges;
   p.qb = p.ranges ? in.nranges : cdiv(in.P, kTblChunk);
   p.grid = p.qb + p.pb + p.nchunks * p.nshares + p.fblocks;
diff --git a/batch-scheduler_amd/csrc/bsched.hip b/batch-scheduler_amd/csrc/bsched.hip
--- a/batch-scheduler_amd/csrc/bsched.hip
+++ b/batch-scheduler_amd/csrc/bsched.hip
@@ -756,6 +756,7 @@
   if (const char* e = std::getenv("BS_TEST_PC_CHUNK_NODES")) c->test_pc_chunk_nodes = (uint32_t)std::max(0, std::atoi(e));
   if (const char* e = std::getenv("BS_STEP_A")) { c->step_a_on = std::atoi(e) != 0; c->step_a_form = (uint32_t)std::atoi(e); }
   if (const char* e = std::getenv("BS_POD_RANGES")) c->pod_ranges_on = std::atoi(e) != 0;
+  if (const char* e = std::getenv("BS_STEP_TABLE")) c->step_table_whole = std::atoi(e) != 0;
   if (const char* e = std::getenv("BS_STEP_SHARES")) c->step_shares = (uint32_t)std::min(32, std::max(1, std::atoi(e)));
   if (const char* e = std::getenv("BS_TP_SHARE")) c->tp_share = (uint32_t)std::min(64, std::max(1, std::atoi(e)));
   if (const char* e = std::getenv("BS_TP_FWAVES")) c->tp_fwaves = (uint32_t)std::max(1, std::atoi(e));
@@ -1592,10 +1593,13 @@
   clock_gettime(CLOCK_MONOTONIC, &ts);
   return (uint64_t)ts.tv_sec * 1000000000ull + (uint64_t)ts.tv_nsec;
 }
-static int step_a_residency(bs_ctx* c, bool whole) {
-  int& r = c->step_a_resident[whole ? 1 : 0];
-  if (r < 0) r = step_a_residency_query(fast_launch(c), whole);
-  return r;
+static int step_a_residency(bs_ctx* c, bool whole, uint32_t table_strips = 0) {
+  int* r = &c->step_a_resident[whole ? 1 : 0];
+  if (whole && table_strips)
+    for (uint32_t i = 0; i < 3; ++i)
+      if (table_strips == kTableWholeStrips[i]) r = &c->step_a_resident_tw[i];
+  if (*r < 0) *r = step_a_residency_query(fast_launch(c), whole, table_strips);
+  return *r;
 }
 
 static BatchParams chain_params(const bs_ctx* c, uint32_t stages, bool use_classes, bool stamped = true) {
@@ -1636,6 +1640,7 @@
   in.whole_bufs = c->d_first_row64.p && c->d_scan_rec.p && c->d_feas_rec.p && c->d_chunk_rec.p;
   in.no_fuse_final = c->no_fuse_final; in.no_nodew = c->no_nodew; in.have_nodew = c->d_nodew.p != nullptr;
   in.collect_stats = c->collect_stats; in.enable_timing = c->cfg.enable_timing;
+  in.table_whole = c->step_table_whole ? 1u : 0u;
   return in;
 }
 
@@ -1715,13 +1720,20 @@
   if (step_a_possible(in, K, nchunks) && (c->step_a_form == 1u || c->dirs_ready || dirs_buildable)) {
     if (c->step_a_form >= 2u && !c->dirs_ready && dirs_buildable && (rc = build_dirs(c))) return rc;
     in.dirs_ready = c->dirs_ready;
-    const StepAPlan pa = step_a_plan(in, K);
+    StepAPlan pa = step_a_plan(in, K);
+    uint32_t strips = pa.table_whole ? table_whole_strips(in.N) : 0u;
+    if (pa.table_whole && !(pa.ready && (int)pa.grid <= step_a_residency(c, true, strips))) {
+      in.table_whole = 0u;
+      pa = step_a_plan(in, K);
+      strips = 0u;
+    }
     if (pa.ranges) b.pod_ranges = c->d_pod_ranges.as<uint32_t>();
-    if (pa.ready && (int)pa.grid <= step_a_residency(c, pa.whole)) {
+    if (pa.ready && (int)pa.grid <= step_a_residency(c, pa.whole, strips)) {
       TIMED(c, BS_KERNEL_QUERY, {
         launch_fast_step_a(fast_launch(c), dim3(pa.grid), pd, gr, nd, b, bt, prm, forced, pa.nchunks, pa.qb, pa.nshares, pa.fblocks, c->tk_pods, c->tk_tab, pa.pb,
-                           c->d_ckeys.as<int64_t>(), c->d_cpres.as<uint32_t>(), c->pair_cap, pa.whole ? 1u : 0u, c->tk_p1, c->tk_done, side_slot - c->C);
+                           c->d_ckeys.as<int64_t>(), c->d_cpres.as<uint32_t>(), c->pair_cap, pa.whole ? 1u : 0u, c->tk_p1, c->tk_done, side_slot - c->C, strips);
       });
+      c->step_form[0] = pa.whole ? 1u : 0u; c->step_form[1] = pa.table_whole ? 1u : 0u; c->step_form[2] = pa.nchunks * pa.nshares; c->step_form[3] = pa.fblocks;
       c->tk_pods += pa.tk_pods;
       c->tk_tab += pa.tk_tab;
       c->tk_p1 += pa.tk_p1;
@@ -1737,6 +1749,7 @@
     }
   }
   c->last_step_a = false;
+  c->step_form[0] = c->step_form[1] = c->step_form[2] = c->step_form[3] = 0u;
   LaunchBPlan pl = launch_b_plan(in);
   if (pl.node_words) {
     b.nodew = bt.nodew = c->d_nodew.as<uint64_t>();
@@ -2182,6 +2195,7 @@
   c->fd_iter = 0;
   c->fd_in_live = false;
   c->batch_void = false;
+  c->step_form[0] = c->step_form[1] = c->step_form[2] = c->step_form[3] = 0u;
   rc = batch_run_inner(c, stages);
   if (rc == BS_OK && (stages & BS_BATCH_FILTER_DENY) && c->P) c->fd_unsynced = true;
   if (rc == BS_OK && (stages & BS_BATCH_FILTER_DENY) && c->P) {
@@ -2847,6 +2861,12 @@
   return BS_OK;
 }
 
+int bs_step_form_get(const bs_ctx* c, uint32_t out[4]) {
+  if (!c || !out) return BS_ERR_INVALID;
+  for (int i = 0; i < 4; ++i) out[i] = c->step_form[i];
+  return BS_OK;
+}
+
 int bs_batch_stats_get(bs_ctx* c, bs_batch_stats* out) {
   if (!c || !out) return BS_ERR_INVALID;
   int rc = use_device(c);
diff --git a/batch-scheduler_amd/csrc/tu_fast.hip b/batch-scheduler_amd/csrc/tu_fast.hip
--- a/batch-scheduler_amd/csrc/tu_fast.hip
+++ b/batch-scheduler_amd/csrc/tu_fast.hip
@@ -52,24 +52,36 @@
   });
 }
 
+template <int TS, class F>
+static auto step_a_strips(uint32_t strips, F&& f) {
+  if (strips == kTableWholeStrips[0]) return f(std::integral_constant<int, (int)kTableWholeStrips[0]>{});
+  if (strips == kTableWholeStrips[1]) return f(std::integral_constant<int, (int)kTableWholeStrips[1]>{});
+  if constexpr (table_whole_strips_max((uint32_t)TS) >= kTableWholeStrips[2])
+    if (strips == kTableWholeStrips[2]) return f(std::integral_constant<int, (int)kTableWholeStrips[2]>{});
+  return f(std::integral_constant<int, 0>{});
+}
+
 void launch_fast_step_a(const FastLaunch& c, dim3 grid, const PodsDev& pd, const GroupsDev& gr, const NodesDev& nd, const BatchDev& b, const BatchDev& bt,
                         const BatchParams& prm, const TableDesc* forced, uint32_t nchunks, uint32_t query_blocks, uint32_t nshares, uint32_t filter_blocks,
                         uint32_t tk_pods0, uint32_t tk_tab0, uint32_t param_blocks, const int64_t* ckeys, const uint32_t* cpres, uint32_t kcap,
-                        uint32_t whole, uint32_t tk_p1, uint32_t tk_done, uint32_t forced_cls) {
+                        uint32_t whole, uint32_t tk_p1, uint32_t tk_done, uint32_t forced_cls, uint32_t table_strips) {
   lanes_clamped(c.S, [&](auto s) {
-    auto launch = [&](auto whole_step) {
-      hipLaunchKernelGGL(HIP_KERNEL_NAME(k_fast_step_a<decltype(s)::value, decltype(whole_step)::value>), grid, dim3(kTblChunk), 0, c.stream, pd, gr, nd, b, bt,
-                         prm, forced, nchunks, query_blocks, nshares, filter_blocks, c.filter_waves, c.filter_slots_cap, tk_pods0, tk_tab0, param_blocks,
-                         ckeys, cpres, kcap, tk_p1, tk_done, forced_cls);
+    auto launch = [&](auto whole_step, auto strips) {
+      hipLaunchKernelGGL(HIP_KERNEL_NAME(k_fast_step_a<decltype(s)::value, decltype(whole_step)::value, decltype(strips)::value>), grid, dim3(kTblChunk), 0, c.stream,
+                         pd, gr, nd, b, bt, prm, forced, nchunks, query_blocks, nshares, filter_blocks, c.filter_waves, c.filter_slots_cap, tk_pods0, tk_tab0,
+                         param_blocks, ckeys, cpres, kcap, tk_p1, tk_done, forced_cls);
     };
-    if (whole) launch(std::true_type{});
-    else launch(std::false_type{});
+    step_a_strips<decltype(s)::value>(whole ? table_strips : 0u, [&](auto strips) {
+      if (whole) launch(std::true_type{}, strips);
+      else launch(std::false_type{}, std::integral_constant<int, 0>{});
+    });
   });
 }
-int step_a_residency_query(const FastLaunch& c, bool whole) {
+int step_a_residency_query(const FastLaunch& c, bool whole, uint32_t table_strips) {
   return lanes_clamped(c.S, [&](auto s) {
     constexpr int TS = decltype(s)::value;
-    return whole ? blocks_resident(c, k_fast_step_a<TS, true>, (int)kTblChunk) : blocks_resident(c, k_fast_step_a<TS, false>, (int)kTblChunk);
+    if (!whole) return blocks_resident(c, k_fast_step_a<TS, false>, (int)kTblChunk);
+    return step_a_strips<TS>(table_strips, [&](auto strips) { return blocks_resident(c, k_fast_step_a<TS, true, decltype(strips)::value>, (int)kTblChunk); });
   });
 }
 
diff --git a/include/bsched.h b/include/bsched.h
--- a/include/bsched.h
+++ b/include/bsched.h
@@ -573,6 +573,7 @@
   uint64_t filter_tile_blocks;
 } bs_batch_stats;
 int bs_batch_stats_get(bs_ctx* ctx, bs_batch_stats* out);
+int bs_step_form_get(const bs_ctx* ctx, uint32_t out[4]);
 int bs_pods_apply_stats(const bs_ctx* ctx, uint64_t* applies, uint64_t* rederives);
 int bs_filter_deny_stats(const bs_ctx* ctx, uint64_t* reruns);
 int bs_speculation_stats(const bs_ctx* ctx, uint64_t* launched, uint64_t* missed);
```

After: 3730 billion evals/s. 0.987x the previous value.
